# c-zhou/oatk

Measured on AMD Instinct MI355X. Metric: HiFi Gbases/s through syncasm (syncmer+syncerr) at k=1001 s=31, higher is better.
Workload: dtype u64

## Files before the change

oatk_amd/csrc/api.hip:

```cpp
#include <hip/hip_runtime.h>
#include <rocprim/device/device_radix_sort.hpp>
#include <rocprim/device/device_scan.hpp>
#include <rocprim/device/device_transform.hpp>
#include <stdio.h>
#include <stdlib.h>
#include <string.h>
#include <time.h>
#include <execinfo.h>
#include <sys/mman.h>
#include <condition_variable>
#include <mutex>
#include <string>
#include <thread>
#include <utility>
#include <vector>

#include "../../include/oatk_hip.h"
#include "common.hpp"
#include "scan_hpc.hpp"
#include "scan_syncmer.hpp"
#include "scan_syncmer_fast.hpp"
#include "kmer_hash.hpp"
#include "count.hpp"

namespace {

static int dev_alloc_log()
{
    static int on = -1;
    if (on < 0) { const char *e = getenv("OATK_DEBUG_ALLOC_LOG"); on = e && e[0] && e[0] != '0'; }
    return on;
}
static double dev_now() { struct timespec t; clock_gettime(CLOCK_MONOTONIC, &t); return (double) t.tv_sec + 1e-9 * (double) t.tv_nsec; }

constexpr size_t DM_CHUNK = 64ull << 20;
static size_t dm_min()
{
    static size_t v = 0;
    if (!v) { const char *e = getenv("OATK_DEBUG_POOL_MIN"); v = e && atoll(e) > 0? (size_t) atoll(e) : (32ull << 20); }
    return v;
}
struct ChunkPool {
    int device = -1;
    bool on = false;
    std::mutex mu;
    std::condition_variable cv;
    std::vector<hipMemGenericAllocationHandle_t> ready;
    std::vector<char> used;
    size_t created = 0, target = 0;
    bool warming = false, stop = false, failed = false;
    std::thread th;
    hipMemAllocationProp prop;
    hipMemAccessDesc acc;
    double t_wait = 0;

    bool create(hipMemGenericAllocationHandle_t *h)
    {
        const double t0 = dev_alloc_log()? dev_now() : 0;
        const hipError_t e = hipMemCreate(h, DM_CHUNK, &prop, 0);
        if (dev_alloc_log() && (e != hipSuccess || dev_now() - t0 > 0.01)) fprintf(stderr, "[oatk alloc] %.3f hipMemCreate %zu MB: %.4f s%s\n", dev_now(), DM_CHUNK >> 20, dev_now() - t0, e == hipSuccess? "" : " FAILED");
        if (e != hipSuccess) (void) hipGetLastError();
        return e == hipSuccess;
    }
    void run()
    {
        (void) hipSetDevice(device);
        for (;;) {
            {
                std::unique_lock<std::mutex> lk(mu);
                if (stop || created >= target) { warming = false; cv.notify_all(); return; }
            }
            hipMemGenericAllocationHandle_t h;
            const bool ok = create(&h);
            std::unique_lock<std::mutex> lk(mu);
            if (!ok) { failed = true, warming = false; cv.notify_all(); return; }
            ready.push_back(h), used.push_back(0), ++created;
            cv.notify_all();
        }
    }
    void warm(size_t bytes)
    {
        size_t fr = 0, tot = 0;
        if (hipMemGetInfo(&fr, &tot) == hipSuccess && bytes > fr / 10 * 7) bytes = fr / 10 * 7;
        std::unique_lock<std::mutex> lk(mu);
        const size_t want = created + bytes / DM_CHUNK;
        if (want > target) target = want;
        if (!warming && !failed && created < target) {
            if (th.joinable()) th.join();
            warming = true;
            th = std::thread([this] { run(); });
        }
    }
    bool take(hipMemGenericAllocationHandle_t *h, bool *was_used)
    {
        *was_used = false;
        {
            std::unique_lock<std::mutex> lk(mu);
            const double t0 = dev_now();
            for (;;) {
                if (!ready.empty()) { *h = ready.back(), *was_used = used.back() != 0; ready.pop_back(), used.pop_back(); t_wait += dev_now() - t0; return true; }
                if (warming && !failed && created < target) { cv.wait(lk); continue; }
                break;
            }
            t_wait += dev_now() - t0;
        }
        if (!create(h)) return false;
        std::unique_lock<std::mutex> lk(mu);
        ++created;
        return true;
    }
    void give(hipMemGenericAllocationHandle_t h)
    {
        std::unique_lock<std::mutex> lk(mu);
        ready.push_back(h), used.push_back(1);
    }
    size_t trim()
    {
        std::unique_lock<std::mutex> lk(mu);
        const size_t n = ready.size();
        for (auto h : ready) (void) hipMemRelease(h);
        ready.clear(), used.clear();
        created -= n, target = created;
        return n;
    }
    void end()
    {
        { std::unique_lock<std::mutex> lk(mu); stop = true; cv.notify_all(); }
        if (th.joinable()) th.join();
    }
};
static ChunkPool *g_pool[64];
static std::mutex g_pool_mu;
static void pools_end() { for (ChunkPool *p : g_pool) if (p) p->end(); }
static ChunkPool *pool_of_current_device()
{
    int d = -1;
    if (hipGetDevice(&d) != hipSuccess || d < 0 || d >= 64) return nullptr;
    ChunkPool *p = g_pool[d];
    return p && p->on? p : nullptr;
}
static ChunkPool *pool_for_new_buffer()
{
    ChunkPool *p = pool_of_current_device();
    if (!p) return nullptr;
    static long lo = -1, hi = -1, seq = 0;
    if (lo < 0) { const char *e = getenv("OATK_DEBUG_POOL_SEQ"); lo = 0, hi = 1L << 60; if (e) sscanf(e, "%ld:%ld", &lo, &hi); }
    const long k = seq++;
    if (dev_alloc_log()) {
        void *bt[6];
        const int nb = backtrace(bt, 6);
        char **sy = backtrace_symbols(bt, nb);
        fprintf(stderr, "[oatk alloc] decision %ld%s  <- %s <- %s <- %s\n", k, k >= lo && k < hi? "" : " (hipMalloc)", nb > 2? sy[2] : "", nb > 3? sy[3] : "", nb > 4? sy[4] : "");
        free(sy);
    }
    return k >= lo && k < hi? p : nullptr;
}

static hipError_t dev_malloc(void **p, size_t bytes)
{
    const double t0 = dev_alloc_log()? dev_now() : 0;
    hipError_t e = hipMalloc(p, bytes);
    if (e != hipSuccess) {
        ChunkPool *pl = pool_of_current_device();
        if (pl && pl->trim()) { (void) hipGetLastError(); e = hipMalloc(p, bytes); }
    }
    if (dev_alloc_log()) fprintf(stderr, "[oatk alloc] %.3f hipMalloc %10.3f MB: %.4f s%s\n", dev_now(), (double) bytes / 1e6, dev_now() - t0, e == hipSuccess? "" : " FAILED");
    {
        static int poison = -1;
        if (poison < 0) { const char *ev = getenv("OATK_DEBUG_POISON"); poison = ev && ev[0] == '1'; }
        if (poison && e == hipSuccess) { (void) hipMemset(*p, 0xA5, bytes); (void) hipDeviceSynchronize(); }
    }
    return e;
}
static void dev_free(void *p, size_t bytes)
{
    const double t0 = dev_alloc_log()? dev_now() : 0;
    (void) hipFree(p);
    if (dev_alloc_log()) fprintf(stderr, "[oatk alloc] %.3f hipFree   %10.3f MB: %.4f s\n", dev_now(), (double) bytes / 1e6, dev_now() - t0);
}

struct DevBuf {
    void *p = nullptr;
    size_t cap = 0;
    size_t va = 0;
    ChunkPool *pool = nullptr;
    bool decided = false;
    std::vector<hipMemGenericAllocationHandle_t> ch;

    static size_t up(size_t b) { return (b + DM_CHUNK - 1) / DM_CHUNK * DM_CHUNK; }
    bool vm_range(size_t bytes, hipStream_t st)
    {
        if (bytes <= va) return true;
        const size_t nva = up(bytes < (1ull << 30)? 4 * bytes + (256ull << 20) : bytes + bytes / 2 + (2ull << 30));
        void *np = nullptr;
        { const hipError_t er = hipMemAddressReserve(&np, nva, 2 << 20, nullptr, 0);
          if (er != hipSuccess) { if (dev_alloc_log()) fprintf(stderr, "[oatk alloc] hipMemAddressReserve of %.1f MB FAILED: %s\n", (double) nva / 1e6, hipGetErrorString(er)); (void) hipGetLastError(); return false; } }
        if (!ch.empty()) {
            (void) hipStreamSynchronize(st);
            (void) hipDeviceSynchronize();
            for (size_t i = 0; i < ch.size(); ++i) {
                (void) hipMemUnmap((char *) p + i * DM_CHUNK, DM_CHUNK);
                if (hipMemMap((char *) np + i * DM_CHUNK, DM_CHUNK, 0, ch[i], 0) != hipSuccess) return false;
            }
            if (hipMemSetAccess(np, ch.size() * DM_CHUNK, &pool->acc, 1) != hipSuccess) return false;
        }
        if (dev_alloc_log()) fprintf(stderr, "[oatk alloc] %.3f address range %10.3f MB (%zu pieces moved)\n", dev_now(), (double) nva / 1e6, ch.size());
        p = np, va = nva;
        return true;
    }
    bool vm_grow(size_t bytes, hipStream_t st)
    {
        const size_t want = up(bytes);
        if (!vm_range(want, st)) return false;
        const size_t have = ch.size() * DM_CHUNK;
        const double t0 = dev_alloc_log()? dev_now() : 0;
        bool any_used = false;
        while (ch.size() * DM_CHUNK < want) {
            hipMemGenericAllocationHandle_t h;
            bool was_used;
            if (!pool->take(&h, &was_used)) { if (dev_alloc_log()) fprintf(stderr, "[oatk alloc] no piece to be had\n"); break; }
            { const hipError_t er = hipMemMap((char *) p + ch.size() * DM_CHUNK, DM_CHUNK, 0, h, 0);
              if (er != hipSuccess) { if (dev_alloc_log()) fprintf(stderr, "[oatk alloc] hipMemMap FAILED: %s\n", hipGetErrorString(er)); (void) hipGetLastError(); pool->give(h); break; } }
            ch.push_back(h);
            any_used |= was_used;
        }
        const size_t now_b = ch.size() * DM_CHUNK;
        if (now_b > have) { const hipError_t er = hipMemSetAccess((char *) p + have, now_b - have, &pool->acc, 1);
                            if (er != hipSuccess) { if (dev_alloc_log()) fprintf(stderr, "[oatk alloc] hipMemSetAccess FAILED: %s\n", hipGetErrorString(er)); (void) hipGetLastError(); return false; } }
        if (any_used && now_b > have && (hipMemsetAsync((char *) p + have, 0, now_b - have, st) != hipSuccess || hipStreamSynchronize(st) != hipSuccess)) return false;
        if (dev_alloc_log()) fprintf(stderr, "[oatk alloc] %.3f pieces    %10.3f MB -> %10.3f MB: %.4f s\n", dev_now(), (double) have / 1e6, (double) now_b / 1e6, dev_now() - t0);
        cap = now_b;
        return now_b >= want;
    }
    bool ensure(size_t bytes, hipStream_t st, bool zero_new = false)
    {
        if (bytes <= cap) return true;
        if (!va && !decided) pool = bytes >= dm_min()? pool_for_new_buffer() : nullptr, decided = bytes >= dm_min();
        if (pool && p && !va) { (void) hipStreamSynchronize(st); dev_free(p, cap); p = nullptr; cap = 0; }
        if (pool) {
            if (vm_grow(bytes + bytes / 16, st)) {
                if (zero_new) (void) hipMemsetAsync(p, 0, cap, st);
                return true;
            }
            if (!ch.empty()) return false;
            pool = nullptr, p = nullptr, cap = 0, va = 0;
        }
        if (p) { (void) hipStreamSynchronize(st); dev_free(p, cap); p = nullptr; cap = 0; }
        size_t want = bytes + bytes / 8 + 256;
        if (dev_malloc(&p, want) != hipSuccess) { p = nullptr; return false; }
        cap = want;
        if (zero_new) (void) hipMemsetAsync(p, 0, want, st);
        return true;
    }
    bool grow_keep(size_t bytes, size_t used, hipStream_t st)
    {
        if (bytes <= cap) return true;
        if (!va && !decided) pool = bytes >= dm_min()? pool_for_new_buffer() : nullptr, decided = bytes >= dm_min();
        if (pool && p && !va) {
            void *old = p;
            const size_t old_cap = cap;
            p = nullptr, cap = 0;
            if (!vm_grow(bytes, st)) { release(); p = old, cap = old_cap, pool = nullptr; }
            else {
                if (used && hipMemcpyAsync(p, old, used, hipMemcpyDeviceToDevice, st) != hipSuccess) return false;
                (void) hipStreamSynchronize(st);
                dev_free(old, old_cap);
                return true;
            }
        }
        if (pool) return vm_grow(bytes, st);
        void *np = nullptr;
        size_t want = bytes + bytes / 4 + 256;
        if (dev_malloc(&np, want) != hipSuccess) return false;
        if (p && used && hipMemcpyAsync(np, p, used, hipMemcpyDeviceToDevice, st) != hipSuccess) { dev_free(np, want); return false; }
        (void) hipStreamSynchronize(st);
        if (p) dev_free(p, cap);
        p = np, cap = want;
        return true;
    }
    bool reserve(size_t bytes, size_t used, hipStream_t st)
    {
        if (bytes <= cap) return true;
        if (!va && !p && !decided) pool = bytes >= dm_min()? pool_for_new_buffer() : nullptr, decided = bytes >= dm_min();
        if (pool && (va || !p)) return vm_range(up(bytes), st);
        return grow_keep(bytes, used, st);
    }
    void release()
    {
        if (va) {
            (void) hipDeviceSynchronize();
            for (size_t i = 0; i < ch.size(); ++i) { (void) hipMemUnmap((char *) p + i * DM_CHUNK, DM_CHUNK); pool->give(ch[i]); }
            ch.clear();
            if (dev_alloc_log()) fprintf(stderr, "[oatk alloc] %.3f pieces    %10.3f MB back to the pool\n", dev_now(), (double) cap / 1e6);
            p = nullptr, cap = 0, va = 0, decided = false;
            return;
        }
        if (p) dev_free(p, cap);
        p = nullptr; cap = 0, decided = false;
    }
    template <class T> T *as() const { return (T *) p; }
};

}

struct oatk_hip_ctx {
    int device = 0;
    int n_cu = 256;
    hipStream_t stream = nullptr;
    std::string err;
    bool timing = false;
    hipEvent_t ev[OATK_T_COUNT_ + 1][2];
    bool ev_used[OATK_T_COUNT_ + 1];
    float ms[OATK_T_COUNT_];
    uint64_t hash_mask = ~0ULL;
    bool force_general = false;
    void *staging = nullptr;
    uint64_t staging_cap = 0;
    void *staging_raw = nullptr;
    uint64_t staging_raw_size = 0;
    bool ra_two_pass = false;
    int list_cap = 0;
    uint64_t import_reserve = 1u << 20;
    int ec_cap_t0 = 0, ec_cap_t1 = 0;

    const uint8_t *d_seq = nullptr;
    const uint64_t *d_off = nullptr;
    const uint32_t *d_len = nullptr;
    DevBuf in_seq, in_off, in_len;
    uint64_t n_reads = 0, seq_bytes = 0, sid0 = 0;
    int K = 0, S = 0;
    bool scanned = false, counted = false;

    DevBuf hoco_l, n_scm, n_nn, n_lrl, ho_rl, hoco_s, nbits;
    DevBuf nn_key, lrl_key, lrl_val, nn_key2, lrl_key2, lrl_val2;
    DevBuf rec_hash, rec_lo, rec_smer, rec_mpos;
    DevBuf raw_lo, raw_smer, raw_mpos, shard_cnt, shard_prefix;
    uint32_t region_cap = 0;
    DevBuf counters;
    uint32_t nn_cap = 0, lrl_cap = 0;
    uint64_t n_occ = 0, tot_nn = 0, tot_lrl = 0, n_scm_total = 0;
    uint32_t retries = 0, collisions = 0;
    bool nn_sorted_in_2 = false, lrl_sorted_in_2 = false;

    DevBuf n_scm64, scm_off, pos_hash, pos_lo, pos_smer, pos_mpos, pos_kid;
    DevBuf key_hash, key_sorted, iota, perm, head, head_idx, newclus, clus_id, bad_head, tag, tmp_perm, flags, kloc, smer_sorted, slot_rec, scm_loc;
    DevBuf scm_h, scm_s, scm_cov, scm_occ_off, scm_occ;
    DevBuf tmp;
    struct EcState *ec = nullptr;
    struct ConsState *cons = nullptr;
    struct IngState *ing = nullptr;
    struct StatState *stat = nullptr;
    struct AgState *ag = nullptr;
    struct OvlState *ovl = nullptr;
    struct RaState *ra = nullptr;
    struct RcState *rc = nullptr;
    struct MultiState *multi = nullptr;
};

#define CK(call)                                                                                   \
    do {                                                                                           \
        hipError_t e_ = (call);                                                                    \
        if (e_ != hipSuccess) {                                                                    \
            ctx->err = std::string(#call) + ": " + hipGetErrorString(e_);                          \
            return OATK_E_NODEV;                                                                   \
        }                                                                                          \
    } while (0)
#define ENSURE(buf, bytes, ...)                                                                    \
    do {                                                                                           \
        if (!ctx->buf.ensure((bytes), ctx->stream, ##__VA_ARGS__)) {                               \
            ctx->err = "hipMalloc failed for " #buf;                                               \
            return OATK_E_NOMEM;                                                                   \
        }                                                                                          \
    } while (0)

static bool debug_refuse(oatk_hip_ctx *ctx, int bit, const char *what)
{
    const char *e = getenv("OATK_DEBUG_REFUSE");
    if (!e || !(atoi(e) & bit)) return false;
    ctx->err = std::string(what) + ": refused on request (OATK_DEBUG_REFUSE)";
    return true;
}

static void t_begin(oatk_hip_ctx *ctx, int which)
{
    if (!ctx->timing) return;
    (void) hipEventRecord(ctx->ev[which][0], ctx->stream);
}
static void t_end(oatk_hip_ctx *ctx, int which)
{
    if (!ctx->timing) return;
    (void) hipEventRecord(ctx->ev[which][1], ctx->stream);
    ctx->ev_used[which] = true;
}
static void t_collect(oatk_hip_ctx *ctx, int first, int last)
{
    if (!ctx->timing) return;
    (void) hipStreamSynchronize(ctx->stream);
    for (int i = first; i <= last; ++i) {
        ctx->ms[i] = 0.f;
        if (ctx->ev_used[i]) (void) hipEventElapsedTime(&ctx->ms[i], ctx->ev[i][0], ctx->ev[i][1]);
        ctx->ev_used[i] = false;
    }
}

#include "api_ec.inc"
#include "api_graph.inc"
#include "api_cons.inc"
#include "api_ovl.inc"
#include "api_align.inc"
#include "api_racov.inc"
#include "api_ingest.inc"
#include "api_stat.inc"
#include "api_multi.inc"
#include "api_multi_tail.inc"

static void staging_free(oatk_hip_ctx *ctx)
{
    if (!ctx->staging) return;
    if (ctx->staging_raw) { (void) hipHostUnregister(ctx->staging); munmap(ctx->staging_raw, ctx->staging_raw_size); }
    else (void) hipHostFree(ctx->staging);
    ctx->staging = ctx->staging_raw = nullptr, ctx->staging_cap = ctx->staging_raw_size = 0;
}

extern "C" {

int oatk_hip_abi_version(void) { return OATK_HIP_ABI_VERSION; }

int oatk_hip_device_count(void)
{
    int n = 0;
    if (hipGetDeviceCount(&n) != hipSuccess) return 0;
    return n;
}

int oatk_hip_max_k(void) { return 8192 - 16 * oatk::SYN_NT - 16 - 64; }

oatk_hip_ctx *oatk_hip_create(int device)
{
    int n = 0;
    if (hipGetDeviceCount(&n) != hipSuccess || device < 0 || device >= n) return nullptr;
    if (hipSetDevice(device) != hipSuccess) return nullptr;
    oatk_hip_ctx *ctx = new oatk_hip_ctx();
    ctx->device = device;
    { int cu = 0; if (hipDeviceGetAttribute(&cu, hipDeviceAttributeMultiprocessorCount, device) == hipSuccess && cu > 0) ctx->n_cu = cu; }
    if (hipStreamCreateWithFlags(&ctx->stream, hipStreamNonBlocking) != hipSuccess) { delete ctx; return nullptr; }
    for (int i = 0; i <= OATK_T_COUNT_; ++i) {
        (void) hipEventCreate(&ctx->ev[i][0]);
        (void) hipEventCreate(&ctx->ev[i][1]);
        ctx->ev_used[i] = false;
    }
    memset(ctx->ms, 0, sizeof(ctx->ms));
    return ctx;
}

void oatk_hip_destroy(oatk_hip_ctx *ctx)
{
    if (!ctx) return;
    (void) hipSetDevice(ctx->device);
    (void) hipStreamSynchronize(ctx->stream);
    DevBuf *all[] = {&ctx->in_seq, &ctx->in_off, &ctx->in_len, &ctx->hoco_l, &ctx->n_scm, &ctx->n_nn, &ctx->n_lrl, &ctx->ho_rl,
                     &ctx->hoco_s, &ctx->nbits, &ctx->nn_key, &ctx->lrl_key, &ctx->lrl_val, &ctx->nn_key2, &ctx->lrl_key2,
                     &ctx->lrl_val2, &ctx->rec_hash, &ctx->rec_lo, &ctx->rec_smer, &ctx->rec_mpos, &ctx->raw_lo, &ctx->raw_smer, &ctx->raw_mpos, &ctx->shard_cnt, &ctx->shard_prefix, &ctx->counters, &ctx->n_scm64,
                     &ctx->scm_off, &ctx->pos_hash, &ctx->pos_lo, &ctx->pos_smer, &ctx->pos_mpos, &ctx->pos_kid, &ctx->key_hash,
                     &ctx->key_sorted, &ctx->iota, &ctx->perm, &ctx->head, &ctx->head_idx, &ctx->newclus, &ctx->clus_id, &ctx->kloc, &ctx->smer_sorted, &ctx->slot_rec, &ctx->scm_loc,
                     &ctx->bad_head, &ctx->tag, &ctx->tmp_perm, &ctx->flags, &ctx->scm_h, &ctx->scm_s, &ctx->scm_cov,
                     &ctx->scm_occ_off, &ctx->scm_occ, &ctx->tmp};
    for (DevBuf *b : all) b->release();
    ec_state_free(ctx);
    cons_state_free(ctx);
    ing_state_free(ctx);
    stat_state_free(ctx);
    ag_state_free(ctx);
    ovl_state_free(ctx);
    ra_state_free(ctx);
    rc_state_free(ctx);
    multi_state_free(ctx);
    for (int i = 0; i <= OATK_T_COUNT_; ++i) {
        (void) hipEventDestroy(ctx->ev[i][0]);
        (void) hipEventDestroy(ctx->ev[i][1]);
    }
    staging_free(ctx);
    (void) hipStreamDestroy(ctx->stream);
    delete ctx;
}

int oatk_hip_mem_pool(oatk_hip_ctx *ctx, uint64_t warm_bytes)
{
    if (!ctx) return OATK_E_NODEV;
    { const char *e = getenv("OATK_POOL"); if (e && e[0] == '0') return OATK_OK; }
    CK(hipSetDevice(ctx->device));
    if (ctx->device < 0 || ctx->device >= 64) return OATK_E_ARG;
    ChunkPool *pl;
    {
        std::unique_lock<std::mutex> lk(g_pool_mu);
        pl = g_pool[ctx->device];
        if (!pl) {
            int vmm = 0;
            if (hipDeviceGetAttribute(&vmm, hipDeviceAttributeVirtualMemoryManagementSupported, ctx->device) != hipSuccess || !vmm) { (void) hipGetLastError(); return OATK_OK; }
            pl = new ChunkPool();
            pl->device = ctx->device;
            memset(&pl->prop, 0, sizeof(pl->prop));
            pl->prop.type = hipMemAllocationTypePinned;
            pl->prop.location.type = hipMemLocationTypeDevice;
            pl->prop.location.id = ctx->device;
            memset(&pl->acc, 0, sizeof(pl->acc));
            pl->acc.location = pl->prop.location;
            pl->acc.flags = hipMemAccessFlagsProtReadWrite;
            static bool at_exit = false;
            if (!at_exit) { at_exit = true; atexit(pools_end); }
            pl->on = true;
            g_pool[ctx->device] = pl;
        }
    }
    if (warm_bytes) pl->warm((size_t) warm_bytes);
    return OATK_OK;
}

const char *oatk_hip_last_error(oatk_hip_ctx *ctx) { return ctx? ctx->err.c_str() : "no device context"; }
void *oatk_hip_stream(oatk_hip_ctx *ctx) { return ctx? (void *) ctx->stream : nullptr; }
int oatk_hip_sync(oatk_hip_ctx *ctx)
{
    if (!ctx) return OATK_E_NODEV;
    CK(hipStreamSynchronize(ctx->stream));
    return OATK_OK;
}
int oatk_hip_set_timing(oatk_hip_ctx *ctx, int enable)
{
    if (!ctx) return OATK_E_NODEV;
    ctx->timing = enable != 0;
    return OATK_OK;
}
int oatk_hip_get_timing(oatk_hip_ctx *ctx, float *ms, int n)
{
    if (!ctx) return OATK_E_NODEV;
    for (int i = 0; i < n && i < OATK_T_COUNT_; ++i) ms[i] = ctx->ms[i];
    return OATK_OK;
}
int oatk_hip_debug_force_general(oatk_hip_ctx *ctx, int on)
{
    if (!ctx) return OATK_E_NODEV;
    ctx->force_general = on != 0;
    return OATK_OK;
}
int oatk_hip_debug_align_two_pass(oatk_hip_ctx *ctx, int on)
{
    if (!ctx) return OATK_E_NODEV;
    ctx->ra_two_pass = on != 0;
    return OATK_OK;
}
int oatk_hip_debug_list_cap(oatk_hip_ctx *ctx, int cap)
{
    if (!ctx) return OATK_E_NODEV;
    if (cap < 0 || cap > oatk::SYF_LIST) { ctx->err = "oatk_hip_debug_list_cap: 0 <= cap <= 128"; return OATK_E_ARG; }
    ctx->list_cap = cap;
    return OATK_OK;
}
int oatk_hip_debug_hash_mask(oatk_hip_ctx *ctx, uint64_t mask)
{
    if (!ctx) return OATK_E_NODEV;
    ctx->hash_mask = mask;
    return OATK_OK;
}

__global__ void widen_kernel(const uint32_t *in, uint64_t *out, uint64_t n)
{
    uint64_t i = (uint64_t) blockIdx.x * blockDim.x + threadIdx.x;
    if (i < n) out[i] = in[i];
    if (i == n) out[i] = 0;
}

static void scan_reset_downstream(oatk_hip_ctx *ctx);

static int launch_scan_kernels(oatk_hip_ctx *ctx)
{
    using namespace oatk;
    const uint64_t n = ctx->n_reads;
    CK(hipMemsetAsync(ctx->counters.p, 0, 4 * sizeof(uint32_t), ctx->stream));
    CK(hipMemsetAsync(ctx->shard_cnt.p, 0, oatk::OATK_REC_SHARDS * sizeof(uint32_t), ctx->stream));
    HpcArgs h;
    h.seq = ctx->d_seq, h.off = ctx->d_off, h.len = ctx->d_len, h.sid0 = ctx->sid0;
    h.ho_rl = ctx->ho_rl.as<uint8_t>(), h.hoco_s = ctx->hoco_s.as<uint8_t>(), h.nbits = ctx->nbits.as<uint32_t>();
    h.hoco_l = ctx->hoco_l.as<uint32_t>(), h.n_nn = ctx->n_nn.as<uint32_t>(), h.n_lrl = ctx->n_lrl.as<uint32_t>();
    h.nn_key = ctx->nn_key.as<uint64_t>(), h.lrl_key = ctx->lrl_key.as<uint64_t>(), h.lrl_val = ctx->lrl_val.as<uint32_t>();
    h.nn_cap = ctx->nn_cap, h.lrl_cap = ctx->lrl_cap, h.counters = ctx->counters.as<uint32_t>();
    t_begin(ctx, OATK_T_HPC);
    h.n_reads = (uint32_t) n;
    constexpr int HPC_NW = 4;
    uint64_t hpc_grid = (uint64_t) ctx->n_cu * 8 * 8;
    { const char *ev = getenv("OATK_DEBUG_HPC_GRID"); if (ev && atoi(ev) > 0) hpc_grid = (uint64_t) atoi(ev); }
    if (hpc_grid * HPC_NW > n) hpc_grid = (n + HPC_NW - 1) / HPC_NW;
    unsigned hpc_dyn = 0;
    { const char *ev = getenv("OATK_DEBUG_HPC_LDS"); if (ev && atoi(ev) > 0) hpc_dyn = (unsigned) atoi(ev); }
    hipLaunchKernelGGL((hpc_pack_kernel<HPC_NW>), dim3((unsigned) (hpc_grid? hpc_grid : 1)), dim3(HPC_NW * OATK_WAVE), hpc_dyn, ctx->stream, h);
    t_end(ctx, OATK_T_HPC);

    SynArgs s;
    s.hoco_s = ctx->hoco_s.as<uint8_t>(), s.nbits = ctx->nbits.as<uint32_t>(), s.off = ctx->d_off;
    s.hoco_l = ctx->hoco_l.as<uint32_t>(), s.n_nn = ctx->n_nn.as<uint32_t>(), s.sid0 = ctx->sid0;
    s.K = ctx->K, s.S = ctx->S, s.want_n = 0, s.n_scm = ctx->n_scm.as<uint32_t>(), s.list_cap = ctx->list_cap? ctx->list_cap : SYF_LIST;
    s.rec_hash = nullptr, s.rec_lo = ctx->raw_lo.as<uint64_t>(), s.rec_smer = ctx->raw_smer.as<uint64_t>();
    s.rec_mpos = ctx->raw_mpos.as<uint32_t>(), s.region_cap = ctx->region_cap, s.shard_cnt = ctx->shard_cnt.as<uint32_t>();
    const bool small = ctx->K + 8 * SYN_NT + 8 + 64 <= 4096;
    const int fast_ring = ctx->force_general? 0 : syncmer_fast_ring(ctx->K, ctx->S);
    t_begin(ctx, OATK_T_SYNCMER);
    if (fast_ring == 4096) {
        const dim3 g((unsigned) n), b(SYN_NT);
        unsigned dyn = 0;
        { const char *ev = getenv("OATK_DEBUG_SYNCMER_LDS"); if (ev && atoi(ev) > 0) dyn = (unsigned) atoi(ev); }
#define OATK_SYF_SWITCH(S31) switch ((-(ctx->K - ctx->S)) & 7) { \
            case 0: OATK_SYF_LAUNCH(S31, 0); break; case 1: OATK_SYF_LAUNCH(S31, 1); break; case 2: OATK_SYF_LAUNCH(S31, 2); break; \
            case 3: OATK_SYF_LAUNCH(S31, 3); break; case 4: OATK_SYF_LAUNCH(S31, 4); break; case 5: OATK_SYF_LAUNCH(S31, 5); break; \
            case 6: OATK_SYF_LAUNCH(S31, 6); break; default: OATK_SYF_LAUNCH(S31, 7); break; }
        const bool two_waves = ctx->K - ctx->S < 1024 && getenv("OATK_DEBUG_SYNCMER_NT256") == nullptr;
#define OATK_SYF_LAUNCH(S31, SH) do { if (two_waves) hipLaunchKernelGGL((syncmer_fast_kernel<2048, S31, 128, SH>), g, dim3(128), dyn, ctx->stream, s); \
                                      else hipLaunchKernelGGL((syncmer_fast_kernel<4096, S31, SYN_NT, SH>), g, b, dyn, ctx->stream, s); } while (0)
        if (ctx->S == 31) OATK_SYF_SWITCH(true) else OATK_SYF_SWITCH(false)
#undef OATK_SYF_SWITCH
#undef OATK_SYF_LAUNCH
    }
    else if (small) hipLaunchKernelGGL((syncmer_kernel<8, 4096, false>), dim3((unsigned) n), dim3(SYN_NT), 0, ctx->stream, s);
    else hipLaunchKernelGGL((syncmer_kernel<16, 8192, false>), dim3((unsigned) n), dim3(SYN_NT), 0, ctx->stream, s);
    t_end(ctx, OATK_T_SYNCMER);
    uint32_t n_amb = 0;
    CK(hipMemcpyAsync(&n_amb, ctx->counters.as<uint32_t>(), 4, hipMemcpyDeviceToHost, ctx->stream));
    CK(hipStreamSynchronize(ctx->stream));
    s.want_n = 1;
    t_begin(ctx, OATK_T_SYNCMER_N);
    if (n_amb) {
        if (small) hipLaunchKernelGGL((syncmer_kernel<8, 4096, true>), dim3((unsigned) n), dim3(SYN_NT), 0, ctx->stream, s);
        else hipLaunchKernelGGL((syncmer_kernel<16, 8192, true>), dim3((unsigned) n), dim3(SYN_NT), 0, ctx->stream, s);
    }
    t_end(ctx, OATK_T_SYNCMER_N);
    CK(hipGetLastError());
    return OATK_OK;
}

int oatk_hip_scan(oatk_hip_ctx *ctx, const uint8_t *d_seq, const uint64_t *d_off, const uint32_t *d_len,
                  uint64_t n_reads, uint64_t seq_bytes, uint64_t sid0, int k, int s)
{
    if (!ctx) return OATK_E_NODEV;
    CK(hipSetDevice(ctx->device));
    if (!(s > 0 && s < 32 && k > s) || k > oatk_hip_max_k()) { ctx->err = "k/s out of range for the device scan"; return OATK_E_ARG; }
    if (seq_bytes % OATK_READ_ALIGN || n_reads >= 0xFFFFFFFFULL || sid0 + n_reads > 0xFFFFFFFFULL) { ctx->err = "bad batch geometry"; return OATK_E_ARG; }
    ctx->d_seq = d_seq, ctx->d_off = d_off, ctx->d_len = d_len;
    ctx->n_reads = n_reads, ctx->seq_bytes = seq_bytes, ctx->sid0 = sid0, ctx->K = k, ctx->S = s;
    scan_reset_downstream(ctx);
    ctx->retries = 0, ctx->collisions = 0;
    ctx->n_occ = ctx->tot_nn = ctx->tot_lrl = ctx->n_scm_total = 0;
    if (n_reads == 0) { ctx->scanned = true; return OATK_OK; }

    ENSURE(hoco_l, n_reads * 4); ENSURE(n_scm, n_reads * 4); ENSURE(n_nn, n_reads * 4); ENSURE(n_lrl, n_reads * 4);
    ENSURE(ho_rl, seq_bytes + 64);
    ENSURE(hoco_s, seq_bytes / 4 + 128 + 16 + ctx->import_reserve);
    ENSURE(nbits, seq_bytes / 8 + 128, true);
    ENSURE(counters, 64);
    if (ctx->nn_cap == 0) ctx->nn_cap = 1u << 14;
    if (ctx->lrl_cap == 0) ctx->lrl_cap = 1u << 14;
    const uint32_t NSH = oatk::OATK_REC_SHARDS;
    {
        uint64_t guess = (seq_bytes / 256 + 1024) / NSH + 256;
        if (ctx->region_cap < guess) ctx->region_cap = (uint32_t) guess;
    }
    ENSURE(shard_cnt, NSH * 4); ENSURE(shard_prefix, NSH * 8);
    uint32_t sc[oatk::OATK_REC_SHARDS];
    uint64_t spfx[oatk::OATK_REC_SHARDS];

    for (;;) {
        const size_t raw_n = (size_t) ctx->region_cap * NSH;
        ENSURE(raw_lo, raw_n * 8); ENSURE(raw_smer, raw_n * 8); ENSURE(raw_mpos, raw_n * 4);
        ENSURE(nn_key, (size_t) ctx->nn_cap * 8); ENSURE(nn_key2, (size_t) ctx->nn_cap * 8);
        ENSURE(lrl_key, (size_t) ctx->lrl_cap * 8); ENSURE(lrl_key2, (size_t) ctx->lrl_cap * 8);
        ENSURE(lrl_val, (size_t) ctx->lrl_cap * 4); ENSURE(lrl_val2, (size_t) ctx->lrl_cap * 4);
        int rc = launch_scan_kernels(ctx);
        if (rc) return rc;
        uint32_t c[4];
        CK(hipMemcpyAsync(c, ctx->counters.p, sizeof(c), hipMemcpyDeviceToHost, ctx->stream));
        CK(hipMemcpyAsync(sc, ctx->shard_cnt.p, sizeof(sc), hipMemcpyDeviceToHost, ctx->stream));
        CK(hipStreamSynchronize(ctx->stream));
        bool again = false;
        if (c[0] > ctx->nn_cap) ctx->nn_cap = c[0] + c[0] / 4, again = true;
        if (c[1] > ctx->lrl_cap) ctx->lrl_cap = c[1] + c[1] / 4, again = true;
        uint64_t tot = 0;
        uint32_t mx = 0;
        for (uint32_t i = 0; i < NSH; ++i) { spfx[i] = tot; tot += sc[i]; if (sc[i] > mx) mx = sc[i]; }
        if (mx > ctx->region_cap) ctx->region_cap = mx + mx / 4 + 16, again = true;
        if (tot > 0xFFFFFFF0ULL) { ctx->err = "more than 2^32 syncmer occurrences in one batch"; return OATK_E_ARG; }
        ctx->tot_nn = c[0], ctx->tot_lrl = c[1], ctx->n_occ = tot;
        if (!again) break;
        ++ctx->retries;
        CK(hipMemsetAsync(ctx->nbits.p, 0, ctx->nbits.cap, ctx->stream));
    }
    if (ctx->n_occ) {
        ENSURE(rec_hash, (size_t) ctx->n_occ * 8); ENSURE(rec_lo, (size_t) ctx->n_occ * 8);
        ENSURE(rec_smer, (size_t) ctx->n_occ * 8); ENSURE(rec_mpos, (size_t) ctx->n_occ * 4);
        CK(hipMemcpyAsync(ctx->shard_prefix.p, spfx, sizeof(spfx), hipMemcpyHostToDevice, ctx->stream));
        oatk::CompactArgs ca;
        ca.raw_lo = ctx->raw_lo.as<uint64_t>(), ca.raw_smer = ctx->raw_smer.as<uint64_t>(), ca.raw_mpos = ctx->raw_mpos.as<uint32_t>();
        ca.shard_cnt = ctx->shard_cnt.as<uint32_t>(), ca.shard_prefix = ctx->shard_prefix.as<uint64_t>(), ca.region_cap = ctx->region_cap;
        ca.rec_lo = ctx->rec_lo.as<uint64_t>(), ca.rec_smer = ctx->rec_smer.as<uint64_t>(), ca.rec_mpos = ctx->rec_mpos.as<uint32_t>();
        hipLaunchKernelGGL(oatk::compact_records_kernel, dim3(NSH), dim3(256), 0, ctx->stream, ca);
        CK(hipStreamSynchronize(ctx->stream));
    }
    if (ctx->timing) t_collect(ctx, OATK_T_HPC, OATK_T_SYNCMER_N);

    if (ctx->n_occ) {
        oatk::KmerHashArgs kh;
        kh.hoco_s = ctx->hoco_s.as<uint8_t>(), kh.off = ctx->d_off, kh.sid0 = ctx->sid0;
        kh.rec_lo = ctx->rec_lo.as<uint64_t>(), kh.rec_mpos = ctx->rec_mpos.as<uint32_t>(), kh.rec_hash = ctx->rec_hash.as<uint64_t>();
        kh.n_rec = (uint32_t) ctx->n_occ, kh.K = ctx->K;
        const int nw = ((ctx->K - 1) / 4 + 1 + 7) / 8;
        t_begin(ctx, OATK_T_KMER_HASH);
        hipLaunchKernelGGL(oatk::kmer_hash_kernel, dim3((unsigned) ((ctx->n_occ + KMH_REC - 1) / KMH_REC)), dim3(64), (size_t) KMH_REC * (nw + 1) * 8, ctx->stream, kh);
        t_end(ctx, OATK_T_KMER_HASH);
    }

    t_begin(ctx, OATK_T_SCAN_POST);
    ctx->nn_sorted_in_2 = ctx->lrl_sorted_in_2 = false;
    if (ctx->tot_nn > 1) {
        size_t tb = 0;
        CK(rocprim::radix_sort_keys(nullptr, tb, ctx->nn_key.as<uint64_t>(), ctx->nn_key2.as<uint64_t>(), ctx->tot_nn, 0, 64, ctx->stream));
        ENSURE(tmp, tb);
        CK(rocprim::radix_sort_keys(ctx->tmp.p, tb, ctx->nn_key.as<uint64_t>(), ctx->nn_key2.as<uint64_t>(), ctx->tot_nn, 0, 64, ctx->stream));
        ctx->nn_sorted_in_2 = true;
    }
    if (ctx->tot_lrl > 1) {
        size_t tb = 0;
        CK(rocprim::radix_sort_pairs(nullptr, tb, ctx->lrl_key.as<uint64_t>(), ctx->lrl_key2.as<uint64_t>(), ctx->lrl_val.as<uint32_t>(),
                                     ctx->lrl_val2.as<uint32_t>(), ctx->tot_lrl, 0, 64, ctx->stream));
        ENSURE(tmp, tb);
        CK(rocprim::radix_sort_pairs(ctx->tmp.p, tb, ctx->lrl_key.as<uint64_t>(), ctx->lrl_key2.as<uint64_t>(), ctx->lrl_val.as<uint32_t>(),
                                     ctx->lrl_val2.as<uint32_t>(), ctx->tot_lrl, 0, 64, ctx->stream));
        ctx->lrl_sorted_in_2 = true;
    }
    {
        ENSURE(n_scm64, (n_reads + 1) * 8); ENSURE(scm_off, (n_reads + 1) * 8);
        unsigned nb = (unsigned) ((n_reads + 1 + 255) / 256);
        hipLaunchKernelGGL(widen_kernel, dim3(nb), dim3(256), 0, ctx->stream, ctx->n_scm.as<uint32_t>(), ctx->n_scm64.as<uint64_t>(), n_reads);
        size_t tb = 0;
        CK(rocprim::exclusive_scan(nullptr, tb, ctx->n_scm64.as<uint64_t>(), ctx->scm_off.as<uint64_t>(), (uint64_t) 0, n_reads + 1,
                                   rocprim::plus<uint64_t>(), ctx->stream));
        ENSURE(tmp, tb);
        CK(rocprim::exclusive_scan(ctx->tmp.p, tb, ctx->n_scm64.as<uint64_t>(), ctx->scm_off.as<uint64_t>(), (uint64_t) 0, n_reads + 1,
                                   rocprim::plus<uint64_t>(), ctx->stream));
    }
    {
        using namespace oatk;
        size_t n = ctx->n_occ? ctx->n_occ : 1;
        ENSURE(pos_hash, n * 8); ENSURE(pos_lo, n * 8); ENSURE(pos_smer, n * 8); ENSURE(pos_mpos, n * 4);
        ENSURE(key_hash, n * 8); ENSURE(iota, n * 4);
        if (ctx->n_occ) {
            PlaceArgs p;
            p.rec_hash = ctx->rec_hash.as<uint64_t>(), p.rec_lo = ctx->rec_lo.as<uint64_t>(), p.rec_smer = ctx->rec_smer.as<uint64_t>();
            p.rec_mpos = ctx->rec_mpos.as<uint32_t>(), p.n_rec = (uint32_t) ctx->n_occ, p.sid0 = ctx->sid0;
            p.scm_off = ctx->scm_off.as<uint64_t>(), p.hash_mask = ctx->hash_mask;
            p.pos_hash = ctx->pos_hash.as<uint64_t>(), p.pos_lo = ctx->pos_lo.as<uint64_t>(), p.pos_smer = ctx->pos_smer.as<uint64_t>();
            p.pos_mpos = ctx->pos_mpos.as<uint32_t>(), p.key_hash = ctx->key_hash.as<uint64_t>(), p.iota = ctx->iota.as<uint32_t>();
            t_begin(ctx, OATK_T_COUNT_PLACE);
            hipLaunchKernelGGL(place_records_kernel, dim3((unsigned) ((ctx->n_occ + 255) / 256)), dim3(256), 0, ctx->stream, p);
            t_end(ctx, OATK_T_COUNT_PLACE);
        }
    }
    t_end(ctx, OATK_T_SCAN_POST);
    CK(hipGetLastError());
    CK(hipStreamSynchronize(ctx->stream));
    if (ctx->timing) { t_collect(ctx, OATK_T_SCAN_POST, OATK_T_COUNT_PLACE); t_collect(ctx, OATK_T_KMER_HASH, OATK_T_KMER_HASH); }
    ctx->scanned = true;
    return OATK_OK;
}

__global__ void append_rebase_kernel(const uint64_t *src, uint64_t *dst, uint64_t n, uint64_t add)
{
    uint64_t i = (uint64_t) blockIdx.x * blockDim.x + threadIdx.x;
    if (i < n) dst[i] = src[i] + add;
}
__global__ void append_iota_kernel(uint32_t *iota, uint64_t first, uint64_t n)
{
    uint64_t i = (uint64_t) blockIdx.x * blockDim.x + threadIdx.x;
    if (i < n) iota[first + i] = (uint32_t) (first + i);
}

static void scan_reset_downstream(oatk_hip_ctx *ctx)
{
    ctx->scanned = ctx->counted = false;
    if (ctx->ec) ctx->ec->done = ctx->ec->marked = ctx->ec->graph_resident = ctx->ec->global = false;
    if (ctx->cons) ctx->cons->done = false;
    if (ctx->ag) ctx->ag->done = false;
    if (ctx->ovl) ctx->ovl->done = false;
    if (ctx->ra) ctx->ra->done = false;
    if (ctx->multi) ctx->multi->merged = ctx->multi->ec_done = false;
}

int oatk_hip_device(oatk_hip_ctx *ctx) { return ctx? ctx->device : -1; }

int oatk_hip_d2d(oatk_hip_ctx *ctx, void *d_dst, const void *d_src, uint64_t bytes)
{
    if (!ctx) return OATK_E_NODEV;
    if (bytes == 0) return OATK_OK;
    CK(hipSetDevice(ctx->device));
    CK(hipMemcpyAsync(d_dst, d_src, bytes, hipMemcpyDeviceToDevice, ctx->stream));
    CK(hipStreamSynchronize(ctx->stream));
    return OATK_OK;
}

int oatk_hip_scan_begin(oatk_hip_ctx *ctx, uint64_t sid0, int k, int s)
{
    if (!ctx) return OATK_E_NODEV;
    CK(hipSetDevice(ctx->device));
    if (!(s > 0 && s < 32 && k > s) || k > oatk_hip_max_k()) { ctx->err = "k/s out of range for the device scan"; return OATK_E_ARG; }
    scan_reset_downstream(ctx);
    ctx->d_seq = nullptr, ctx->d_off = nullptr, ctx->d_len = nullptr;
    ctx->n_reads = 0, ctx->seq_bytes = 0, ctx->sid0 = sid0, ctx->K = k, ctx->S = s;
    ctx->retries = 0, ctx->collisions = 0;
    ctx->n_occ = ctx->tot_nn = ctx->tot_lrl = ctx->n_scm_total = 0;
    ctx->nn_sorted_in_2 = ctx->lrl_sorted_in_2 = false;
    ctx->scanned = true;
    return OATK_OK;
}

#define KEEP(buf, bytes, used)                                                                     \
    do {                                                                                           \
        if (!ctx->buf.grow_keep((bytes), (used), ctx->stream)) {                                   \
            ctx->err = "hipMalloc failed for " #buf " (append)";                                   \
            return OATK_E_NOMEM;                                                                   \
        }                                                                                          \
    } while (0)

static int append_ensure(oatk_hip_ctx *ctx, uint64_t nr, uint64_t sb, uint64_t occ, uint64_t nn, uint64_t lrl)
{
    const uint64_t n0 = ctx->n_reads, b0 = ctx->seq_bytes, o0 = ctx->n_occ;
    KEEP(in_off, (nr + 1) * 8, n0 * 8);
    KEEP(hoco_l, nr * 4 + 4, n0 * 4); KEEP(n_scm, nr * 4 + 4, n0 * 4); KEEP(n_nn, nr * 4 + 4, n0 * 4); KEEP(n_lrl, nr * 4 + 4, n0 * 4);
    KEEP(ho_rl, sb + 64, b0);
    KEEP(hoco_s, sb / 4 + 128 + 16 + ctx->import_reserve, b0 / 4 + 64);
    KEEP(scm_off, (nr + 1) * 8, (n0 + 1) * 8);
    KEEP(pos_hash, occ * 8 + 8, o0 * 8); KEEP(pos_lo, occ * 8 + 8, o0 * 8); KEEP(pos_smer, occ * 8 + 8, o0 * 8); KEEP(pos_mpos, occ * 4 + 4, o0 * 4);
    KEEP(key_hash, occ * 8 + 8, o0 * 8); KEEP(iota, occ * 4 + 4, o0 * 4);
    KEEP(nn_key, nn * 8 + 8, ctx->tot_nn * 8); KEEP(lrl_key, lrl * 8 + 8, ctx->tot_lrl * 8); KEEP(lrl_val, lrl * 4 + 4, ctx->tot_lrl * 4);
    return OATK_OK;
}

int oatk_hip_scan_reserve(oatk_hip_ctx *ctx, uint64_t seq_bytes, uint64_t n_reads, uint64_t n_occ)
{
    if (!ctx) return OATK_E_NODEV;
    CK(hipSetDevice(ctx->device));
    if (!ctx->scanned || ctx->d_seq) { ctx->err = "oatk_hip_scan_reserve: call oatk_hip_scan_begin first"; return OATK_E_STATE; }
    seq_bytes = (seq_bytes + 63) & ~63ULL;
    if (pool_of_current_device()) {
        const uint64_t sb = ctx->seq_bytes + seq_bytes;
        if (!ctx->ho_rl.reserve(sb + 64, ctx->seq_bytes, ctx->stream) || !ctx->hoco_s.reserve(sb / 4 + 128 + 16 + ctx->import_reserve, ctx->seq_bytes / 4 + 64, ctx->stream)) {
            ctx->err = "oatk_hip_scan_reserve: no address range for the batch";
            return OATK_E_NOMEM;
        }
        return OATK_OK;
    }
    return append_ensure(ctx, ctx->n_reads + n_reads, ctx->seq_bytes + seq_bytes, ctx->n_occ + n_occ, ctx->tot_nn, ctx->tot_lrl);
}

int oatk_hip_scan_append(oatk_hip_ctx *ctx, oatk_hip_ctx *src)
{
    if (!ctx || !src) return OATK_E_NODEV;
    CK(hipSetDevice(ctx->device));
    if (ctx == src || ctx->device != src->device) { ctx->err = "oatk_hip_scan_append: the piece must be another handle on the same device"; return OATK_E_ARG; }
    if (!ctx->scanned || ctx->d_seq) { ctx->err = "oatk_hip_scan_append: call oatk_hip_scan_begin first"; return OATK_E_STATE; }
    if (!src->scanned) { ctx->err = "oatk_hip_scan_append: the piece holds no scan"; return OATK_E_STATE; }
    const uint64_t n0 = ctx->n_reads, n1 = src->n_reads, b0 = ctx->seq_bytes, b1 = src->seq_bytes, o0 = ctx->n_occ, o1 = src->n_occ;
    if (n1 == 0) return OATK_OK;
    if (src->K != ctx->K || src->S != ctx->S) { ctx->err = "oatk_hip_scan_append: the piece was scanned with another k / s"; return OATK_E_ARG; }
    if (src->sid0 != ctx->sid0 + n0) { ctx->err = "oatk_hip_scan_append: the piece's first read id must continue the batch"; return OATK_E_ARG; }
    if (n0 + n1 >= 0xFFFFFFFFULL || o0 + o1 > 0xFFFFFFF0ULL) { ctx->err = "oatk_hip_scan_append: batch too large"; return OATK_E_ARG; }
    scan_reset_downstream(ctx);
    ctx->scanned = true;
    { int rc = append_ensure(ctx, n0 + n1, b0 + b1, o0 + o1, ctx->tot_nn + src->tot_nn, ctx->tot_lrl + src->tot_lrl); if (rc) return rc; }
    if (hipStreamSynchronize(src->stream) != hipSuccess) { ctx->err = "oatk_hip_scan_append: the piece's stream failed"; return OATK_E_NODEV; }
    hipStream_t st = ctx->stream;
    auto blocks = [](uint64_t n) { return dim3((unsigned) ((n + 255) / 256 > 0? (n + 255) / 256 : 1)); };
    auto d2d = [&](void *dst, const void *from, size_t bytes) { return bytes? hipMemcpyAsync(dst, from, bytes, hipMemcpyDeviceToDevice, st) : hipSuccess; };
    CK(d2d(ctx->ho_rl.as<uint8_t>() + b0, src->ho_rl.p, b1));
    CK(d2d(ctx->hoco_s.as<uint8_t>() + b0 / 4, src->hoco_s.p, b1 / 4 + 64));
    CK(d2d(ctx->hoco_l.as<uint32_t>() + n0, src->hoco_l.p, n1 * 4)); CK(d2d(ctx->n_scm.as<uint32_t>() + n0, src->n_scm.p, n1 * 4));
    CK(d2d(ctx->n_nn.as<uint32_t>() + n0, src->n_nn.p, n1 * 4)); CK(d2d(ctx->n_lrl.as<uint32_t>() + n0, src->n_lrl.p, n1 * 4));
    hipLaunchKernelGGL(append_rebase_kernel, blocks(n1), dim3(256), 0, st, src->d_off, ctx->in_off.as<uint64_t>() + n0, n1, b0);
    hipLaunchKernelGGL(append_rebase_kernel, blocks(n1 + 1), dim3(256), 0, st, src->scm_off.as<uint64_t>(), ctx->scm_off.as<uint64_t>() + n0, n1 + 1, o0);
    if (o1) {
        CK(d2d(ctx->pos_hash.as<uint64_t>() + o0, src->pos_hash.p, o1 * 8)); CK(d2d(ctx->pos_lo.as<uint64_t>() + o0, src->pos_lo.p, o1 * 8));
        CK(d2d(ctx->pos_smer.as<uint64_t>() + o0, src->pos_smer.p, o1 * 8)); CK(d2d(ctx->pos_mpos.as<uint32_t>() + o0, src->pos_mpos.p, o1 * 4));
        CK(d2d(ctx->key_hash.as<uint64_t>() + o0, src->key_hash.p, o1 * 8));
        hipLaunchKernelGGL(append_iota_kernel, blocks(o1), dim3(256), 0, st, ctx->iota.as<uint32_t>(), o0, o1);
    }
    CK(d2d(ctx->nn_key.as<uint64_t>() + ctx->tot_nn, src->nn_sorted_in_2? src->nn_key2.p : src->nn_key.p, src->tot_nn * 8));
    CK(d2d(ctx->lrl_key.as<uint64_t>() + ctx->tot_lrl, src->lrl_sorted_in_2? src->lrl_key2.p : src->lrl_key.p, src->tot_lrl * 8));
    CK(d2d(ctx->lrl_val.as<uint32_t>() + ctx->tot_lrl, src->lrl_sorted_in_2? src->lrl_val2.p : src->lrl_val.p, src->tot_lrl * 4));
    CK(hipGetLastError());
    CK(hipStreamSynchronize(st));
    ctx->d_off = ctx->in_off.as<uint64_t>();
    ctx->n_reads = n0 + n1, ctx->seq_bytes = b0 + b1, ctx->n_occ = o0 + o1;
    ctx->tot_nn += src->tot_nn, ctx->tot_lrl += src->tot_lrl;
    ctx->retries += src->retries;
    return OATK_OK;
}

int oatk_hip_scan_host(oatk_hip_ctx *ctx, const uint8_t *h_seq, const uint64_t *h_off, const uint32_t *h_len,
                       uint64_t n_reads, uint64_t seq_bytes, uint64_t sid0, int k, int s)
{
    if (!ctx) return OATK_E_NODEV;
    CK(hipSetDevice(ctx->device));
    ENSURE(in_seq, seq_bytes + 64); ENSURE(in_off, (n_reads + 1) * 8); ENSURE(in_len, (n_reads + 1) * 4);
    if (seq_bytes) CK(hipMemcpyAsync(ctx->in_seq.p, h_seq, seq_bytes, hipMemcpyHostToDevice, ctx->stream));
    if (n_reads) {
        CK(hipMemcpyAsync(ctx->in_off.p, h_off, n_reads * 8, hipMemcpyHostToDevice, ctx->stream));
        CK(hipMemcpyAsync(ctx->in_len.p, h_len, n_reads * 4, hipMemcpyHostToDevice, ctx->stream));
    }
    return oatk_hip_scan(ctx, ctx->in_seq.as<uint8_t>(), ctx->in_off.as<uint64_t>(), ctx->in_len.as<uint32_t>(), n_reads, seq_bytes, sid0, k, s);
}

int oatk_hip_count(oatk_hip_ctx *ctx)
{
    using namespace oatk;
    if (!ctx) return OATK_E_NODEV;
    if (!ctx->scanned) { ctx->err = "count before scan"; return OATK_E_STATE; }
    CK(hipSetDevice(ctx->device));
    ctx->counted = false;
    ctx->n_scm_total = 0;
    if (ctx->multi) ctx->multi->merged = ctx->multi->ec_done = false;
    const uint64_t n = ctx->n_occ;
    if (n == 0) { ctx->counted = true; return OATK_OK; }
    const unsigned nb = (unsigned) ((n + 255) / 256);

    ENSURE(key_sorted, n * 8); ENSURE(perm, n * 4); ENSURE(head, n * 4); ENSURE(head_idx, n * 4); ENSURE(newclus, n * 4); ENSURE(kloc, n * 8);
    if (ctx->seq_bytes >> 4 >= 0xFFFFFFFFULL) { ctx->err = "batch too large for 32-bit hoco word indices (64 GB of bases)"; return OATK_E_ARG; }
    ENSURE(clus_id, n * 4); ENSURE(bad_head, n * 4); ENSURE(tag, n * 4); ENSURE(tmp_perm, n * 4); ENSURE(flags, 64);
    ENSURE(pos_kid, n * 8); ENSURE(scm_occ, n * 8);
    CK(hipMemsetAsync(ctx->flags.p, 0, 64, ctx->stream));

    bool full_sort = getenv("OATK_DEBUG_FULL_SORT") != nullptr || n < (1ull << 22);
sort_again:
    t_begin(ctx, OATK_T_COUNT_SORT);
    {
        const unsigned lo_bit = full_sort? 0u : (unsigned) OATK_SORT_LOW_BITS;
        size_t tb = 0;
        CK(rocprim::radix_sort_pairs(nullptr, tb, ctx->key_hash.as<uint64_t>(), ctx->key_sorted.as<uint64_t>(), ctx->iota.as<uint32_t>(),
                                     ctx->perm.as<uint32_t>(), n, lo_bit, 64, ctx->stream));
        ENSURE(tmp, tb);
        CK(rocprim::radix_sort_pairs(ctx->tmp.p, tb, ctx->key_hash.as<uint64_t>(), ctx->key_sorted.as<uint64_t>(), ctx->iota.as<uint32_t>(),
                                     ctx->perm.as<uint32_t>(), n, lo_bit, 64, ctx->stream));
        if (!full_sort) {
            uint32_t *owner = ctx->head.as<uint32_t>();
            CK(hipMemsetAsync(owner, 0xFF, n * 4, ctx->stream));
            hipLaunchKernelGGL(sort_repair_find_kernel, dim3(nb), dim3(256), 0, ctx->stream, ctx->key_sorted.as<uint64_t>(), (uint32_t) n, owner, ctx->flags.as<uint32_t>());
            hipLaunchKernelGGL(sort_repair_kernel, dim3(nb), dim3(256), 0, ctx->stream, ctx->key_sorted.as<uint64_t>(), ctx->perm.as<uint32_t>(), (uint32_t) n, owner,
                               ctx->flags.as<uint32_t>());
        }
    }
    t_end(ctx, OATK_T_COUNT_SORT);

    t_begin(ctx, OATK_T_COUNT_GROUP);
    GroupArgs g;
    g.sorted_key = ctx->key_sorted.as<uint64_t>(), g.perm = ctx->perm.as<uint32_t>(), g.n_rec = (uint32_t) n;
    g.pos_lo = ctx->pos_lo.as<uint64_t>(), g.pos_mpos = ctx->pos_mpos.as<uint32_t>(), g.hoco_s = ctx->hoco_s.as<uint8_t>();
    g.off = ctx->d_off, g.sid0 = ctx->sid0, g.K = ctx->K;
    g.head = ctx->head.as<uint32_t>(), g.head_idx = ctx->head_idx.as<uint32_t>(), g.newclus = ctx->newclus.as<uint32_t>();
    g.loc = ctx->kloc.as<uint64_t>();
    ENSURE(smer_sorted, n * 8);
    g.pos_smer = ctx->pos_smer.as<uint64_t>(), g.occ_sorted = ctx->scm_occ.as<uint64_t>(), g.smer_sorted = ctx->smer_sorted.as<uint64_t>();
    g.flags = ctx->flags.as<uint32_t>();
    ENSURE(slot_rec, n * 32);
    g.slot_rec = ctx->slot_rec.as<uint4>();
    hipLaunchKernelGGL(pack_slots_kernel, dim3(nb), dim3(256), 0, ctx->stream, g);
    hipLaunchKernelGGL(pair_sum_kernel, dim3(2048), dim3(256), 0, ctx->stream, ctx->key_hash.as<uint64_t>(), (const uint32_t *) nullptr, (uint32_t) n, ctx->flags.as<uint32_t>(), 8);
    hipLaunchKernelGGL(pair_sum_kernel, dim3(2048), dim3(256), 0, ctx->stream, ctx->key_sorted.as<uint64_t>(), ctx->perm.as<uint32_t>(), (uint32_t) n, ctx->flags.as<uint32_t>(), 12);
    hipLaunchKernelGGL(heads_only_kernel, dim3(nb), dim3(256), 0, ctx->stream, g);
    {
        size_t tb = 0;
        CK(rocprim::inclusive_scan(nullptr, tb, ctx->head_idx.as<uint32_t>(), ctx->head_idx.as<uint32_t>(), n, rocprim::maximum<uint32_t>(), ctx->stream));
        ENSURE(tmp, tb);
        CK(rocprim::inclusive_scan(ctx->tmp.p, tb, ctx->head_idx.as<uint32_t>(), ctx->head_idx.as<uint32_t>(), n, rocprim::maximum<uint32_t>(), ctx->stream));
    }
    uint32_t n_scm = 0;
    FinishArgs f;
    auto ids = [&]() -> int {
        size_t tb = 0;
        CK(rocprim::inclusive_scan(nullptr, tb, ctx->newclus.as<uint32_t>(), ctx->clus_id.as<uint32_t>(), n, rocprim::plus<uint32_t>(), ctx->stream));
        ENSURE(tmp, tb);
        CK(rocprim::inclusive_scan(ctx->tmp.p, tb, ctx->newclus.as<uint32_t>(), ctx->clus_id.as<uint32_t>(), n, rocprim::plus<uint32_t>(), ctx->stream));
        uint32_t last_id = 0;
        CK(hipMemcpyAsync(&last_id, ctx->clus_id.as<uint32_t>() + (n - 1), 4, hipMemcpyDeviceToHost, ctx->stream));
        CK(hipStreamSynchronize(ctx->stream));
        n_scm = last_id;
        ENSURE(scm_h, (size_t) n_scm * 8); ENSURE(scm_s, (size_t) n_scm * 8); ENSURE(scm_cov, (size_t) n_scm * 4); ENSURE(scm_loc, (size_t) n_scm * 8);
        ENSURE(scm_occ_off, ((size_t) n_scm + 1) * 8);
        f.perm = ctx->perm.as<uint32_t>(), f.newclus = ctx->newclus.as<uint32_t>(), f.clus_id = ctx->clus_id.as<uint32_t>(), f.n_rec = (uint32_t) n;
        f.sorted_key = ctx->key_sorted.as<uint64_t>(), f.smer_sorted = ctx->smer_sorted.as<uint64_t>();
        f.loc = ctx->kloc.as<uint64_t>(), f.scm_loc = ctx->scm_loc.as<uint64_t>();
        f.scm_h = ctx->scm_h.as<uint64_t>(), f.scm_s = ctx->scm_s.as<uint64_t>(), f.scm_occ_off = ctx->scm_occ_off.as<uint64_t>();
        f.scm_occ = ctx->scm_occ.as<uint64_t>(), f.pos_kid = ctx->pos_kid.as<uint64_t>(), f.flags = ctx->flags.as<uint32_t>();
        return OATK_OK;
    };
    { int rc = ids(); if (rc) return rc; }
    hipLaunchKernelGGL(gather_finish_kernel, dim3(nb), dim3(256), 0, ctx->stream, g, f, ctx->clus_id.as<uint32_t>(), n_scm);
    CK(hipMemsetAsync(ctx->bad_head.p, 0, n * 4, ctx->stream));
    hipLaunchKernelGGL(verify_group_kernel, dim3((unsigned) ((n + 8 * OATK_VG_STRIP - 1) / (8 * OATK_VG_STRIP))), dim3(256), 0, ctx->stream, g, ctx->bad_head.as<uint32_t>());
    CK(rocprim::transform(ctx->clus_id.as<uint32_t>(), ctx->clus_id.as<uint32_t>(), n, [] __device__(uint32_t v) { return v - 1u; }, ctx->stream));
    uint32_t fl[16];
    CK(hipMemcpyAsync(fl, ctx->flags.p, sizeof(fl), hipMemcpyDeviceToHost, ctx->stream));
    CK(hipStreamSynchronize(ctx->stream));
    const bool sort_bad = fl[4] != 0 || memcmp(fl + 8, fl + 12, 16) != 0 || (!full_sort && getenv("OATK_DEBUG_SORT_DISTRUST") != nullptr);
    if (sort_bad && full_sort) {
        t_end(ctx, OATK_T_COUNT_GROUP);
        ctx->err = "the device sort returned something that is not its input in order (rocPRIM radix_sort_pairs): refusing to build the syncmer table from it";
        return OATK_E_NODEV;
    }
    if ((fl[3] || sort_bad) && !full_sort) {
        t_end(ctx, OATK_T_COUNT_GROUP);
        CK(hipMemsetAsync(ctx->flags.p, 0, 64, ctx->stream));
        full_sort = true;
        goto sort_again;
    }
    if (fl[0]) {
        ctx->collisions = 1;
        hipLaunchKernelGGL(split_collisions_kernel, dim3(nb), dim3(256), 0, ctx->stream, g, ctx->bad_head.as<uint32_t>(), ctx->perm.as<uint32_t>(),
                           ctx->tag.as<uint32_t>(), ctx->tmp_perm.as<uint32_t>());
        hipLaunchKernelGGL(regather_kernel, dim3(nb), dim3(256), 0, ctx->stream, g);
        { int rc = ids(); if (rc) return rc; }
        CK(rocprim::transform(ctx->clus_id.as<uint32_t>(), ctx->clus_id.as<uint32_t>(), n, [] __device__(uint32_t v) { return v - 1u; }, ctx->stream));
        hipLaunchKernelGGL(finish_heads_kernel, dim3(nb), dim3(256), 0, ctx->stream, f, n_scm);
    }
    hipLaunchKernelGGL(check_smer_kernel, dim3(nb), dim3(256), 0, ctx->stream, f);
    hipLaunchKernelGGL(cov_kernel, dim3((n_scm + 255) / 256), dim3(256), 0, ctx->stream, ctx->scm_occ_off.as<uint64_t>(), ctx->scm_cov.as<uint32_t>(), n_scm);
    t_end(ctx, OATK_T_COUNT_GROUP);
    CK(hipGetLastError());
    CK(hipMemcpyAsync(fl, ctx->flags.p, sizeof(fl), hipMemcpyDeviceToHost, ctx->stream));
    CK(hipStreamSynchronize(ctx->stream));
    if (ctx->timing) t_collect(ctx, OATK_T_COUNT_SORT, OATK_T_COUNT_GROUP);
    if (fl[2]) { ctx->err = "hash group with too many distinct k-mers"; return OATK_E_SPLIT; }
    if (debug_refuse(ctx, 4, "oatk_hip_count")) return OATK_E_SPLIT;
    if (fl[1]) { ctx->err = "identical kmers have different smers"; return OATK_E_SMER; }
    ctx->n_scm_total = n_scm;
    ctx->counted = true;
    return OATK_OK;
}

int oatk_hip_info(oatk_hip_ctx *ctx, oatk_hip_info_t *out)
{
    if (!ctx) return OATK_E_NODEV;
    out->n_reads = ctx->n_reads, out->seq_bytes = ctx->seq_bytes, out->sid0 = ctx->sid0;
    out->k = ctx->K, out->s = ctx->S;
    out->n_occ = ctx->n_occ, out->n_nn = ctx->tot_nn, out->n_lrl = ctx->tot_lrl;
    out->n_scm = ctx->n_scm_total;
    out->scan_retries = ctx->retries, out->collisions = ctx->collisions;
    return OATK_OK;
}

int oatk_hip_buffer(oatk_hip_ctx *ctx, int which, const void **d_ptr, uint64_t *bytes)
{
    if (!ctx) return OATK_E_NODEV;
    if (which >= OATK_BUF_INGEST_SEQ && which <= OATK_BUF_INGEST_HDR) return ing_buffer(ctx, which, d_ptr, bytes);
    if (which >= OATK_BUF_MG_H && which <= OATK_BUF_MG_LCOV) return multi_buffer(ctx, which, d_ptr, bytes);
    if (which >= OATK_BUF_MG_G_H && which <= OATK_BUF_MG_POS_GKID) return multi_tail_buffer(ctx, which, d_ptr, bytes);
    if (!ctx->scanned) { ctx->err = "no resident scan"; return OATK_E_STATE; }
    const uint64_t n = ctx->n_reads, occ = ctx->n_occ, ns = ctx->n_scm_total;
    const void *p = nullptr;
    uint64_t b = 0;
    switch (which) {
        case OATK_BUF_HOCO_L: p = ctx->hoco_l.p, b = n * 4; break;
        case OATK_BUF_N_SCM: p = ctx->n_scm.p, b = n * 4; break;
        case OATK_BUF_N_NN: p = ctx->n_nn.p, b = n * 4; break;
        case OATK_BUF_N_LRL: p = ctx->n_lrl.p, b = n * 4; break;
        case OATK_BUF_HO_RL: p = ctx->ho_rl.p, b = ctx->seq_bytes; break;
        case OATK_BUF_HOCO_S: p = ctx->hoco_s.p, b = ctx->seq_bytes / 4 + 64; break;
        case OATK_BUF_NN_KEY: p = ctx->nn_sorted_in_2? ctx->nn_key2.p : ctx->nn_key.p, b = ctx->tot_nn * 8; break;
        case OATK_BUF_LRL_KEY: p = ctx->lrl_sorted_in_2? ctx->lrl_key2.p : ctx->lrl_key.p, b = ctx->tot_lrl * 8; break;
        case OATK_BUF_LRL_VAL: p = ctx->lrl_sorted_in_2? ctx->lrl_val2.p : ctx->lrl_val.p, b = ctx->tot_lrl * 4; break;
        case OATK_BUF_SCM_OFF: p = ctx->scm_off.p, b = (n + 1) * 8; break;
        case OATK_BUF_POS_MPOS: p = ctx->pos_mpos.p, b = occ * 4; break;
        case OATK_BUF_POS_SMER: p = ctx->pos_smer.p, b = occ * 8; break;
        case OATK_BUF_POS_HASH: p = ctx->pos_hash.p, b = occ * 8; break;
        default:
            if (!ctx->counted) { ctx->err = "count results requested before oatk_hip_count"; return OATK_E_STATE; }
            switch (which) {
                case OATK_BUF_POS_KID: p = ctx->pos_kid.p, b = occ * 8; break;
                case OATK_BUF_SCM_H: p = ctx->scm_h.p, b = ns * 8; break;
                case OATK_BUF_SCM_S: p = ctx->scm_s.p, b = ns * 8; break;
                case OATK_BUF_SCM_COV: p = ctx->scm_cov.p, b = ns * 4; break;
                case OATK_BUF_SCM_OCC_OFF: p = ctx->scm_occ_off.p, b = (ns + 1) * 8; break;
                case OATK_BUF_SCM_OCC: p = ctx->scm_occ.p, b = occ * 8; break;
                default:
                    if (which >= OATK_BUF_CONS_SEL && which <= OATK_BUF_CONS_TOT) return cons_buffer(ctx, which, d_ptr, bytes);
                    if (which >= OATK_BUF_AG_SCM_DEL && which <= OATK_BUF_AG_ARC_LINK) return ag_buffer(ctx, which, d_ptr, bytes);
                    if (which >= OATK_BUF_OVL_KEY && which <= OATK_BUF_OVL_TAIL) return ovl_buffer(ctx, which, d_ptr, bytes);
                    if (which >= OATK_BUF_RA_ALN_SID && which <= OATK_BUF_RA_SKIPPED) return ra_buffer(ctx, which, d_ptr, bytes);
                    if (which >= OATK_BUF_INGEST_SEQ && which <= OATK_BUF_INGEST_HDR) return ing_buffer(ctx, which, d_ptr, bytes);
                    return ec_buffer(ctx, which, d_ptr, bytes);
            }
    }
    *d_ptr = p, *bytes = b;
    return OATK_OK;
}

void *oatk_hip_staging(oatk_hip_ctx *ctx, uint64_t bytes)
{
    if (!ctx || hipSetDevice(ctx->device) != hipSuccess) return nullptr;
    if (bytes <= ctx->staging_cap) return ctx->staging;
    staging_free(ctx);
    const uint64_t HP = 2ull << 20, want = (bytes + HP - 1) & ~(HP - 1);
    void *raw = mmap(nullptr, want + HP, PROT_READ | PROT_WRITE, MAP_PRIVATE | MAP_ANONYMOUS, -1, 0);
    if (raw != MAP_FAILED) {
        uint8_t *base = (uint8_t *) (((uintptr_t) raw + HP - 1) & ~(uintptr_t) (HP - 1));
        (void) madvise(base, want, MADV_HUGEPAGE);
        const int nt = want >= (256ull << 20)? 8 : 1;
        std::vector<std::thread> th;
        for (int t = 1; t < nt; ++t) th.emplace_back([=] { for (uint64_t o = want / nt * t; o < (t + 1 == nt? want : want / nt * (t + 1)); o += 4096) *(volatile uint8_t *) (base + o) = 0; });
        for (uint64_t o = 0; o < want / nt; o += 4096) *(volatile uint8_t *) (base + o) = 0;
        for (auto &x : th) x.join();
        if (hipHostRegister(base, want, hipHostRegisterDefault) == hipSuccess) {
            ctx->staging = base, ctx->staging_cap = want, ctx->staging_raw = raw, ctx->staging_raw_size = want + HP;
            return ctx->staging;
        }
        (void) hipGetLastError();
        munmap(raw, want + HP);
    }
    if (hipHostMalloc(&ctx->staging, bytes, hipHostMallocDefault) != hipSuccess) { ctx->staging = nullptr; ctx->err = "hipHostMalloc failed (staging)"; return nullptr; }
    ctx->staging_cap = bytes;
    return ctx->staging;
}

int oatk_hip_host_register(oatk_hip_ctx *ctx, void *p, uint64_t bytes)
{
    if (!ctx) return OATK_E_NODEV;
    if (!p || bytes == 0) return OATK_E_ARG;
    CK(hipSetDevice(ctx->device));
    CK(hipHostRegister(p, bytes, hipHostRegisterDefault));
    return OATK_OK;
}

int oatk_hip_host_unregister(oatk_hip_ctx *ctx, void *p)
{
    if (!ctx) return OATK_E_NODEV;
    CK(hipSetDevice(ctx->device));
    CK(hipHostUnregister(p));
    return OATK_OK;
}

int oatk_hip_d2h(oatk_hip_ctx *ctx, void *h_dst, const void *d_src, uint64_t bytes)
{
    if (!ctx) return OATK_E_NODEV;
    if (bytes == 0) return OATK_OK;
    CK(hipSetDevice(ctx->device));
    CK(hipMemcpyAsync(h_dst, d_src, bytes, hipMemcpyDeviceToHost, ctx->stream));
    CK(hipStreamSynchronize(ctx->stream));
    return OATK_OK;
}

int oatk_hip_d2h_async(oatk_hip_ctx *ctx, void *h_dst, const void *d_src, uint64_t bytes)
{
    if (!ctx) return OATK_E_NODEV;
    if (bytes == 0) return OATK_OK;
    CK(hipSetDevice(ctx->device));
    CK(hipMemcpyAsync(h_dst, d_src, bytes, hipMemcpyDeviceToHost, ctx->stream));
    return OATK_OK;
}

int oatk_hip_h2d_async(oatk_hip_ctx *ctx, void *d_dst, const void *h_src, uint64_t bytes)
{
    if (!ctx) return OATK_E_NODEV;
    if (bytes == 0) return OATK_OK;
    CK(hipSetDevice(ctx->device));
    CK(hipMemcpyAsync(d_dst, h_src, bytes, hipMemcpyHostToDevice, ctx->stream));
    return OATK_OK;
}

}
```

oatk_amd/csrc/common.hpp:

```cpp
#pragma once
#include <hip/hip_runtime.h>
#include <stdint.h>

#define OATK_WAVE 64

namespace oatk {

__device__ __forceinline__ uint32_t nt4_code(uint32_t ch)
{
    uint32_t up = ch & 0xDFu;
    uint32_t t = up - 0x41u;
    bool letter = t < 32u && ((0x00180045u >> t) & 1u);
    uint32_t code = (up >> 1) & 3u;
    code ^= code >> 1;
    return ch < 4u ? ch : (letter ? code : 4u);
}

__device__ __forceinline__ uint64_t hash64(uint64_t x, uint64_t mask)
{
    x = (~x + (x << 21)) & mask;
    x ^= x >> 24;
    x = (x + (x << 3) + (x << 8)) & mask;
    x ^= x >> 14;
    x = (x + (x << 2) + (x << 4)) & mask;
    x ^= x >> 28;
    x = (x + (x << 31)) & mask;
    return x;
}

__device__ __forceinline__ uint64_t hash64_s31(uint64_t x)
{
    uint32_t lo = (uint32_t) x, hi = (uint32_t) (x >> 32);
    uint64_t p;
    p = (uint64_t) lo * 0x1FFFFFu + 0xFFFFFFFFFFFFFFFFull;
    hi = (uint32_t) (p >> 32) + (hi << 21) - hi, lo = (uint32_t) p;
    { const uint32_t t = __builtin_amdgcn_alignbit(hi, lo, 24), u = __builtin_amdgcn_ubfe(hi, 24, 6); lo ^= t, hi ^= u; }
    p = (uint64_t) lo * 265u;
    hi = hi * 265u + (uint32_t) (p >> 32), lo = (uint32_t) p;
    { const uint32_t t = __builtin_amdgcn_alignbit(hi, lo, 14), u = __builtin_amdgcn_ubfe(hi, 14, 16); lo ^= t, hi ^= u; }
    p = (uint64_t) hi << 32 | lo;
    {
        uint64_t p5;
        asm("v_lshl_add_u64 %0, %1, 2, %1" : "=v"(p5) : "v"(p));
        asm("v_lshl_add_u64 %0, %1, 4, %2" : "=v"(p) : "v"(p), "v"(p5));
    }
    hi = (uint32_t) (p >> 32), lo = (uint32_t) p;
    { const uint32_t t = __builtin_amdgcn_alignbit(hi, lo, 28), u = __builtin_amdgcn_ubfe(hi, 28, 2); lo ^= t, hi ^= u; }
    p = (uint64_t) lo * 0x80000001u;
    hi = (hi + (uint32_t) (p >> 32)) & 0x3FFFFFFFu, lo = (uint32_t) p;
    return (uint64_t) hi << 32 | lo;
}

__device__ __forceinline__ uint64_t hash64_s31_left(uint64_t x4)
{
    uint32_t lo = (uint32_t) x4 & ~3u, hi = (uint32_t) (x4 >> 32);
    uint64_t p;
    p = (uint64_t) lo * 0x1FFFFFu + 0xFFFFFFFFFFFFFFFCull;
    hi = (uint32_t) (p >> 32) + (hi << 21) - hi, lo = (uint32_t) p;
    { const uint32_t t = __builtin_amdgcn_alignbit(hi, lo, 24) & ~3u, u = hi >> 24; lo ^= t, hi ^= u; }
    p = (uint64_t) lo * 265u;
    hi = hi * 265u + (uint32_t) (p >> 32), lo = (uint32_t) p;
    { const uint32_t t = __builtin_amdgcn_alignbit(hi, lo, 14) & ~3u, u = hi >> 14; lo ^= t, hi ^= u; }
    p = (uint64_t) hi << 32 | lo;
    {
        uint64_t p5;
        asm("v_lshl_add_u64 %0, %1, 2, %1" : "=v"(p5) : "v"(p));
        asm("v_lshl_add_u64 %0, %1, 4, %2" : "=v"(p) : "v"(p), "v"(p5));
    }
    hi = (uint32_t) (p >> 32), lo = (uint32_t) p;
    { const uint32_t t = __builtin_amdgcn_alignbit(hi, lo, 28) & ~3u, u = hi >> 28; lo ^= t, hi ^= u; }
    hi += __builtin_amdgcn_alignbit(hi, lo, 1);
    return (uint64_t) hi << 32 | lo;
}

__device__ __forceinline__ uint64_t revcomp32(uint64_t x)
{
    uint32_t lo = (uint32_t) x, hi = (uint32_t) (x >> 32);
    uint32_t rlo = __builtin_bitreverse32(hi), rhi = __builtin_bitreverse32(lo);
    uint64_t r = (uint64_t) rhi << 32 | rlo;
    r = ((r >> 1) & 0x5555555555555555ULL) | ((r & 0x5555555555555555ULL) << 1);
    return ~r;
}

__device__ __forceinline__ uint64_t bswap64(uint64_t x) { return __builtin_bswap64(x); }

#define OATK_MURMUR_M 0xc6a4a7935bd1e995ULL
#define OATK_MURMUR_SEED 1234ULL

__device__ __forceinline__ uint64_t murmur_mix_word(uint64_t w)
{
    w *= OATK_MURMUR_M;
    w ^= w >> 47;
    w *= OATK_MURMUR_M;
    return w;
}

__device__ __forceinline__ uint32_t wave_incl_sum(uint32_t v, int lane)
{
#pragma unroll
    for (int d = 1; d < OATK_WAVE; d <<= 1) {
        uint32_t o = __shfl_up(v, d);
        if (lane >= d) v += o;
    }
    return v;
}

__device__ __forceinline__ int32_t wave_incl_max(int32_t v, int lane)
{
#pragma unroll
    for (int d = 1; d < OATK_WAVE; d <<= 1) {
        int32_t o = __shfl_up(v, d);
        if (lane >= d) v = v > o? v : o;
    }
    return v;
}

}
```

oatk_amd/csrc/count.hpp:

```cpp
#pragma once
#include "common.hpp"

namespace oatk {

struct CompactArgs {
    const uint64_t *raw_lo, *raw_smer;
    const uint32_t *raw_mpos;
    const uint32_t *shard_cnt;
    const uint64_t *shard_prefix;
    uint32_t region_cap;
    uint64_t *rec_lo, *rec_smer;
    uint32_t *rec_mpos;
};

__global__ __launch_bounds__(256) void compact_records_kernel(CompactArgs a)
{
    const uint32_t sh = blockIdx.x, n = a.shard_cnt[sh];
    const size_t src = (size_t) sh * a.region_cap;
    const uint64_t dst = a.shard_prefix[sh];
    for (uint32_t i = threadIdx.x; i < n; i += blockDim.x) {
        a.rec_lo[dst + i] = a.raw_lo[src + i];
        a.rec_smer[dst + i] = a.raw_smer[src + i];
        a.rec_mpos[dst + i] = a.raw_mpos[src + i];
    }
}

struct PlaceArgs {
    const uint64_t *rec_hash, *rec_lo, *rec_smer;
    const uint32_t *rec_mpos;
    uint32_t n_rec;
    uint64_t sid0;
    const uint64_t *scm_off;
    uint64_t hash_mask;
    uint64_t *pos_hash, *pos_lo, *pos_smer;
    uint32_t *pos_mpos;
    uint64_t *key_hash;
    uint32_t *iota;
};

__global__ void place_records_kernel(PlaceArgs a)
{
    uint32_t i = blockIdx.x * blockDim.x + threadIdx.x;
    if (i >= a.n_rec) return;
    uint64_t lo = a.rec_lo[i];
    uint64_t rd = (lo >> 32) - a.sid0;
    uint64_t p = a.scm_off[rd] + ((uint32_t) lo >> 1);
    a.pos_hash[p] = a.rec_hash[i];
    a.key_hash[p] = a.rec_hash[i] & a.hash_mask;
    a.pos_lo[p] = lo;
    a.pos_smer[p] = a.rec_smer[i];
    a.pos_mpos[p] = a.rec_mpos[i];
    a.iota[p] = (uint32_t) p;
}

__device__ __forceinline__ uint64_t kmer_word_global(const uint32_t *hs32, uint32_t pos, uint32_t rev, int K, int wd)
{
    int32_t t = rev? (int32_t) pos + K - 32 - 32 * wd : (int32_t) pos + 32 * wd;
    int nb = K - 32 * wd;
    nb = nb > 32? 32 : nb;
    int32_t wi = t >> 4;
    uint32_t sh = ((uint32_t) t & 15u) * 2u;
    uint32_t w0, w1, w2;
    if (wi >= 0) {
        struct __attribute__((packed, aligned(4))) W3 { uint32_t a, b, c; };
        const W3 v = *(const W3 *) (hs32 + wi);
        w0 = __builtin_bswap32(v.a), w1 = __builtin_bswap32(v.b), w2 = __builtin_bswap32(v.c);
    } else {
        w0 = 0u;
        w1 = wi + 1 >= 0? __builtin_bswap32(hs32[wi + 1]) : 0u;
        w2 = wi + 2 >= 0? __builtin_bswap32(hs32[wi + 2]) : 0u;
    }
    uint64_t hi = (uint64_t) w0 << 32 | w1;
    uint64_t V = sh? (hi << sh) | ((uint64_t) w2 >> (32u - sh)) : hi;
    if (rev) V = revcomp32(V);
    if (nb < 32) V &= ~0ULL << (64 - 2 * nb);
    return V;
}

struct GroupArgs {
    const uint64_t *sorted_key;
    const uint32_t *perm;
    uint32_t n_rec;
    const uint64_t *pos_lo;
    const uint32_t *pos_mpos;
    const uint8_t *hoco_s;
    const uint64_t *off;
    uint64_t sid0;
    int K;
    uint32_t *head;
    uint32_t *head_idx;
    uint32_t *newclus;
    uint32_t *flags;
    uint64_t *loc;
    const uint64_t *pos_smer;
    uint64_t *occ_sorted, *smer_sorted;
    uint4 *slot_rec;
};

__global__ void pack_slots_kernel(GroupArgs a)
{
    uint32_t p = blockIdx.x * blockDim.x + threadIdx.x;
    if (p >= a.n_rec) return;
    const uint64_t lo = a.pos_lo[p], sm = a.pos_smer[p];
    const uint64_t loc = ((a.off[(lo >> 32) - a.sid0] >> 4) << 32) | a.pos_mpos[p];
    a.slot_rec[2 * (size_t) p] = make_uint4((uint32_t) lo, (uint32_t) (lo >> 32), (uint32_t) sm, (uint32_t) (sm >> 32));
    a.slot_rec[2 * (size_t) p + 1] = make_uint4((uint32_t) loc, (uint32_t) (loc >> 32), 0u, 0u);
}

#define OATK_SORT_LOW_BITS 24
#define OATK_SORT_REPAIR_MAX 4096u
__device__ __forceinline__ bool sort_repair_boundary(const uint64_t *key, uint32_t n, uint32_t i, uint32_t &start, uint32_t *flags)
{
    if (i == 0 || i >= n) return false;
    const uint64_t k = key[i], kp = key[i - 1];
    if ((k >> OATK_SORT_LOW_BITS) != (kp >> OATK_SORT_LOW_BITS) || k == kp) return false;
    uint32_t s = i - 1;
    while (s > 0 && (key[s - 1] >> OATK_SORT_LOW_BITS) == (k >> OATK_SORT_LOW_BITS)) {
        --s;
        if (i - s > OATK_SORT_REPAIR_MAX) { flags[3] = 1u; return false; }
    }
    start = s;
    return true;
}
__global__ void sort_repair_find_kernel(const uint64_t *key, uint32_t n, uint32_t *owner, uint32_t *flags)
{
    const uint32_t i = blockIdx.x * blockDim.x + threadIdx.x;
    uint32_t s;
    if (sort_repair_boundary(key, n, i, s, flags)) atomicMin(&owner[s], i);
    if (i > 0 && i < n && (key[i] >> OATK_SORT_LOW_BITS) < (key[i - 1] >> OATK_SORT_LOW_BITS)) flags[3] = 1u;
}
__global__ void sort_repair_kernel(uint64_t *key, uint32_t *perm, uint32_t n, uint32_t *owner, uint32_t *flags)
{
    const uint32_t i = blockIdx.x * blockDim.x + threadIdx.x;
    uint32_t s;
    if (!sort_repair_boundary(key, n, i, s, flags) || owner[s] != i) return;
    const uint64_t top = key[i] >> OATK_SORT_LOW_BITS;
    uint32_t e = i + 1;
    while (e < n && (key[e] >> OATK_SORT_LOW_BITS) == top) {
        ++e;
        if (e - s > OATK_SORT_REPAIR_MAX) { flags[3] = 1u; return; }
    }
    for (uint32_t a = i; a < e; ++a) {
        const uint64_t kk = key[a];
        const uint32_t pp = perm[a];
        uint32_t b = a;
        while (b > s && key[b - 1] > kk) { key[b] = key[b - 1], perm[b] = perm[b - 1]; --b; }
        key[b] = kk, perm[b] = pp;
    }
}

__device__ __forceinline__ void pair_sums(uint64_t key, uint32_t slot, uint64_t &s0, uint64_t &s1)
{
    uint64_t x = key ^ ((uint64_t) slot * 0x9E3779B97F4A7C15ULL);
    x ^= x >> 32; x *= 0xD6E8FEB86659FD93ULL; x ^= x >> 32;
    s0 = x;
    x *= 0xD6E8FEB86659FD93ULL; x ^= x >> 29; x += key;
    s1 = x;
}
__global__ __launch_bounds__(256) void pair_sum_kernel(const uint64_t *key, const uint32_t *perm, uint32_t n, uint32_t *flags, int at)
{
    __shared__ uint64_t part[2][4];
    uint64_t s0 = 0, s1 = 0;
    bool inv = false;
    const uint64_t stride = (uint64_t) gridDim.x * blockDim.x;
    for (uint64_t i0 = (uint64_t) blockIdx.x * blockDim.x + threadIdx.x; i0 < n; i0 += 4 * stride) {
        uint64_t k[4], kp[4];
        uint32_t v[4];
#pragma unroll
        for (int u = 0; u < 4; ++u) {
            const uint64_t i = i0 + u * stride;
            const bool in = i < n;
            k[u] = in? key[i] : 0, v[u] = in? (perm? perm[i] : (uint32_t) i) : 0, kp[u] = in && perm && i? key[i - 1] : 0;
        }
#pragma unroll
        for (int u = 0; u < 4; ++u) {
            if (i0 + u * stride >= n) continue;
            uint64_t a, b;
            pair_sums(k[u], v[u], a, b);
            s0 += a, s1 += b;
            if (k[u] < kp[u]) inv = true;
        }
    }
    #pragma unroll
    for (int d = 32; d > 0; d >>= 1) s0 += __shfl_xor(s0, d), s1 += __shfl_xor(s1, d);
    if ((threadIdx.x & 63u) == 0) part[0][threadIdx.x >> 6] = s0, part[1][threadIdx.x >> 6] = s1;
    if (inv) flags[4] = 1u;
    __syncthreads();
    if (threadIdx.x == 0) {
        atomicAdd((unsigned long long *) (flags + at), (unsigned long long) (part[0][0] + part[0][1] + part[0][2] + part[0][3]));
        atomicAdd((unsigned long long *) (flags + at + 2), (unsigned long long) (part[1][0] + part[1][1] + part[1][2] + part[1][3]));
    }
}

__global__ void heads_only_kernel(GroupArgs a)
{
    uint32_t i = blockIdx.x * blockDim.x + threadIdx.x;
    if (i >= a.n_rec) return;
    const uint32_t h = i == 0 || a.sorted_key[i] != a.sorted_key[i - 1];
    a.head[i] = h;
    a.newclus[i] = h;
    a.head_idx[i] = h? i : 0u;
}

__global__ void mark_heads_kernel(GroupArgs a)
{
    uint32_t i = blockIdx.x * blockDim.x + threadIdx.x;
    if (i >= a.n_rec) return;
    uint32_t h = i == 0 || a.sorted_key[i] != a.sorted_key[i - 1];
    a.head[i] = h;
    a.newclus[i] = h;
    a.head_idx[i] = h? i : 0u;
    const uint32_t p = a.perm[i];
    const uint4 r0 = a.slot_rec[2 * (size_t) p], r1 = a.slot_rec[2 * (size_t) p + 1];
    a.loc[i] = (uint64_t) r1.y << 32 | r1.x;
    a.occ_sorted[i] = (uint64_t) r0.y << 32 | r0.x, a.smer_sorted[i] = (uint64_t) r0.w << 32 | r0.z;
}
__global__ void regather_kernel(GroupArgs a)
{
    uint32_t i = blockIdx.x * blockDim.x + threadIdx.x;
    if (i >= a.n_rec) return;
    const uint32_t p = a.perm[i];
    const uint4 r0 = a.slot_rec[2 * (size_t) p], r1 = a.slot_rec[2 * (size_t) p + 1];
    a.loc[i] = (uint64_t) r1.y << 32 | r1.x;
    a.occ_sorted[i] = (uint64_t) r0.y << 32 | r0.x, a.smer_sorted[i] = (uint64_t) r0.w << 32 | r0.z;
}

#ifndef OATK_VG_STRIP
#define OATK_VG_STRIP 8
#endif
#ifndef OATK_VFY_WAVES
#define OATK_VFY_WAVES 1
#endif
__global__ __launch_bounds__(256, OATK_VFY_WAVES) void verify_group_kernel(GroupArgs a, uint32_t *bad_head)
{
    const uint32_t hl = threadIdx.x & 31, half0 = threadIdx.x & 32;
    const uint32_t i0 = (uint32_t) OATK_VG_STRIP * (blockIdx.x * (blockDim.x >> 5) + (threadIdx.x >> 5));
    uint32_t my_h = 0;
    uint64_t my_lp = 0, my_lq = 0;
    bool my_live = false;
    if (hl < OATK_VG_STRIP) {
        const uint32_t i = i0 + hl;
        my_live = i < a.n_rec && !a.head[i];
        if (my_live) {
            my_h = a.head_idx[i];
            my_lp = a.loc[i];
            my_lq = a.loc[my_h];
        }
    }
    const uint64_t live_mask = (__ballot(my_live) >> half0) & ((1ULL << OATK_VG_STRIP) - 1ULL);
    if (live_mask == 0) return;
    const uint32_t *hs32 = (const uint32_t *) a.hoco_s;
    const int nw = (a.K + 31) / 32;
    uint32_t diff = 0;
    const uint32_t first_live = (uint32_t) __builtin_ctzll(live_mask);
    const uint64_t lq0 = (uint64_t) __shfl((long long) my_lq, (int) (half0 + first_live));
    const bool one_head = __ballot(my_live && my_lq != lq0) == 0;
    for (int w0 = 0; w0 < nw; w0 += 32) {
        const int wd = w0 + (int) hl;
        const bool in = wd < nw;
        uint64_t p[OATK_VG_STRIP], q[OATK_VG_STRIP];
        if (one_head) {
            const uint64_t q0 = in? kmer_word_global(hs32 + (lq0 >> 32), (uint32_t) lq0 >> 1, (uint32_t) lq0 & 1u, a.K, wd) : 0;
#pragma unroll
            for (int r = 0; r < OATK_VG_STRIP; ++r) {
                const uint64_t lp = (uint64_t) __shfl((long long) my_lp, (int) (half0 + r));
                const bool live = in && ((live_mask >> r) & 1u);
                p[r] = live? kmer_word_global(hs32 + (lp >> 32), (uint32_t) lp >> 1, (uint32_t) lp & 1u, a.K, wd) : q0;
            }
#pragma unroll
            for (int r = 0; r < OATK_VG_STRIP; ++r) diff |= (uint32_t) (p[r] != q0) << r;
        } else {
#pragma unroll
            for (int r = 0; r < OATK_VG_STRIP; ++r) {
                const uint64_t lp = (uint64_t) __shfl((long long) my_lp, (int) (half0 + r)), lq = (uint64_t) __shfl((long long) my_lq, (int) (half0 + r));
                const bool live = in && ((live_mask >> r) & 1u);
                p[r] = live? kmer_word_global(hs32 + (lp >> 32), (uint32_t) lp >> 1, (uint32_t) lp & 1u, a.K, wd) : 0;
                q[r] = live? kmer_word_global(hs32 + (lq >> 32), (uint32_t) lq >> 1, (uint32_t) lq & 1u, a.K, wd) : 0;
            }
#pragma unroll
            for (int r = 0; r < OATK_VG_STRIP; ++r) diff |= (uint32_t) (p[r] != q[r]) << r;
        }
    }
#pragma unroll
    for (int r = 0; r < OATK_VG_STRIP; ++r) {
        const uint64_t bad = (__ballot((diff >> r) & 1u) >> half0) & 0xFFFFFFFFULL;
        if (bad && hl == (uint32_t) r) a.flags[0] = 1u, bad_head[my_h] = 1u;
    }
}

#define OATK_MAX_SPLIT 16
__global__ void split_collisions_kernel(GroupArgs a, const uint32_t *bad_head, uint32_t *perm_rw, uint32_t *tag, uint32_t *tmp_perm)
{
    uint32_t i = blockIdx.x * blockDim.x + threadIdx.x;
    if (i >= a.n_rec || !a.head[i] || !bad_head[i]) return;
    uint32_t e = i + 1;
    while (e < a.n_rec && !a.head[e]) ++e;
    const int nw = (a.K + 31) / 32;
    uint32_t rep[OATK_MAX_SPLIT], nclus = 0;
    for (uint32_t t = i; t < e; ++t) {
        uint32_t p = perm_rw[t];
        uint64_t lo_p = a.pos_lo[p];
        const uint32_t *hs_p = (const uint32_t *) (a.hoco_s + (a.off[(lo_p >> 32) - a.sid0] >> 2));
        uint32_t mp = a.pos_mpos[p], c;
        for (c = 0; c < nclus; ++c) {
            uint32_t q = perm_rw[rep[c]];
            uint64_t lo_q = a.pos_lo[q];
            const uint32_t *hs_q = (const uint32_t *) (a.hoco_s + (a.off[(lo_q >> 32) - a.sid0] >> 2));
            uint32_t mq = a.pos_mpos[q];
            bool same = true;
            for (int wd = 0; wd < nw && same; ++wd)
                same = kmer_word_global(hs_p, mp >> 1, mp & 1u, a.K, wd) == kmer_word_global(hs_q, mq >> 1, mq & 1u, a.K, wd);
            if (same) break;
        }
        if (c == nclus) {
            if (nclus == OATK_MAX_SPLIT) { a.flags[2] = 1u; return; }
            rep[nclus++] = t;
        }
        tag[t] = c;
    }
    uint32_t w = i;
    for (uint32_t c = 0; c < nclus; ++c) {
        bool first = true;
        for (uint32_t t = i; t < e; ++t)
            if (tag[t] == c) {
                tmp_perm[w] = perm_rw[t];
                a.newclus[w] = first? 1u : 0u;
                first = false;
                ++w;
            }
    }
    for (uint32_t t = i; t < e; ++t) perm_rw[t] = tmp_perm[t];
}

struct FinishArgs {
    const uint32_t *perm;
    const uint32_t *newclus;
    const uint32_t *clus_id;
    uint32_t n_rec;
    const uint64_t *sorted_key, *smer_sorted;
    uint64_t *scm_h, *scm_s;
    uint64_t *scm_occ_off;
    uint64_t *scm_occ;
    const uint64_t *loc;
    uint64_t *scm_loc;
    uint64_t *pos_kid;
    uint32_t *flags;
};

__global__ void finish_heads_kernel(FinishArgs a, uint32_t n_scm)
{
    uint32_t i = blockIdx.x * blockDim.x + threadIdx.x;
    if (i >= a.n_rec) return;
    uint32_t p = a.perm[i], id = a.clus_id[i];
    a.pos_kid[p] = (uint64_t) id << 1;
    if (a.newclus[i]) {
        a.scm_h[id] = a.sorted_key[i];
        a.scm_s[id] = a.smer_sorted[i];
        a.scm_occ_off[id] = i;
        a.scm_loc[id] = a.loc[i];
    }
    if (i == a.n_rec - 1) a.scm_occ_off[n_scm] = a.n_rec;
}

__global__ void gather_finish_kernel(GroupArgs g, FinishArgs a, const uint32_t *clus_id1, uint32_t n_scm)
{
    uint32_t i = blockIdx.x * blockDim.x + threadIdx.x;
    if (i >= a.n_rec) return;
    const uint32_t p = g.perm[i], id = clus_id1[i] - 1u;
    const uint4 r0 = g.slot_rec[2 * (size_t) p], r1 = g.slot_rec[2 * (size_t) p + 1];
    const uint64_t loc = (uint64_t) r1.y << 32 | r1.x, smer = (uint64_t) r0.w << 32 | r0.z;
    g.loc[i] = loc;
    g.occ_sorted[i] = (uint64_t) r0.y << 32 | r0.x, g.smer_sorted[i] = smer;
    a.pos_kid[p] = (uint64_t) id << 1;
    if (g.newclus[i]) {
        a.scm_h[id] = a.sorted_key[i];
        a.scm_s[id] = smer;
        a.scm_occ_off[id] = i;
        a.scm_loc[id] = loc;
    }
    if (i == a.n_rec - 1) a.scm_occ_off[n_scm] = a.n_rec;
}

__global__ void check_smer_kernel(FinishArgs a)
{
    uint32_t i = blockIdx.x * blockDim.x + threadIdx.x;
    if (i >= a.n_rec) return;
    uint32_t id = a.clus_id[i];
    if (a.smer_sorted[i] != a.scm_s[id]) a.flags[1] = 1u;
}

__global__ void cov_kernel(const uint64_t *occ_off, uint32_t *cov, uint32_t n_scm)
{
    uint32_t i = blockIdx.x * blockDim.x + threadIdx.x;
    if (i < n_scm) cov[i] = (uint32_t) (occ_off[i + 1] - occ_off[i]);
}

}
```

oatk_amd/csrc/ec.hpp:

```cpp
#pragma once
#include "common.hpp"

namespace oatk {

#define EC_FAILURE 0
#define EC_SUCCESS 1
#define EC_AMBISNQ 2
#define EC_AMBISEQ 3
#define EC_MAX_DFS_PATH 10000
#define EC_MIN_ERR_SEQ_LEN 10
#define EC_MIN_ERR_BASE 6
#define EC_NONE 0xFFFFFFFFFFFFFFFFULL

struct EcGraph {
    uint64_t n_vtx, n_arc;
    const uint64_t *idx_p;
    const uint32_t *idx_n;
    const uint64_t *arc_v, *arc_w;
    const uint32_t *arc_ls, *arc_cov;
    uint8_t *arc_del;
    uint8_t *scm_del;
    const uint32_t *scm_cov;
    const uint64_t *scm_s;
    const uint64_t *vtx_hs_off;
    const uint32_t *vtx_mpos;
    const uint8_t *other;
};

struct EcReads {
    uint64_t n_reads, sid0;
    int K;
    const uint8_t *hoco_s;
    const uint64_t *off;
    const uint32_t *hoco_l;
    const uint64_t *scm_off;
    const uint64_t *k_mer;
    const uint32_t *m_pos;
};

__global__ void ec_mark_kernel(EcGraph g, uint32_t err_mer_c, uint32_t max_err_c, uint32_t err_arc_c, double max_arc_f)
{
    uint64_t i = (uint64_t) blockIdx.x * blockDim.x + threadIdx.x;
    if (i >= g.n_vtx) return;
    if (g.scm_del[i] || g.scm_cov[i] >= max_err_c) return;
    if (g.scm_cov[i] < err_mer_c) { g.scm_del[i] = 1; return; }
    const uint32_t nv = g.scm_cov[i];
    int b[2] = {-1, -1};
    for (int k = 0; k < 2; ++k) {
        const uint64_t v = i << 1 | (uint64_t) k, p = g.idx_p[v];
        const uint32_t na = g.idx_n[v];
        uint32_t live = 0;
        for (uint32_t j = 0; j < na; ++j) live += !g.arc_del[p + j];
        if (!live && !(g.other && g.other[v])) continue;
        b[k] = 0;
        for (uint32_t j = 0; j < na; ++j) {
            if (g.arc_del[p + j]) continue;
            const uint32_t nw = g.scm_cov[g.arc_w[p + j] >> 1], mn = nv < nw? nv : nw, ac = g.arc_cov[p + j];
            if (ac >= err_arc_c && (double) ac >= (double) mn * max_arc_f) { b[k] = 1; break; }
        }
    }
    if (!b[0] || !b[1]) g.scm_del[i] = 1;
}

__global__ void ec_arc_del_kernel(EcGraph g)
{
    uint64_t a = (uint64_t) blockIdx.x * blockDim.x + threadIdx.x;
    if (a >= g.n_arc) return;
    if (g.scm_del[g.arc_v[a] >> 1] || g.scm_del[g.arc_w[a] >> 1]) g.arc_del[a] = 1;
}

#define EC_NO_SRC 0xFFFFFFFFFFFFFFFFULL
__global__ void ec_vtx_src_kernel(uint64_t n_local, const uint64_t *scm_loc, const uint32_t *l2g, uint64_t *vtx_hs_off, uint32_t *vtx_mpos)
{
    uint64_t i = (uint64_t) blockIdx.x * blockDim.x + threadIdx.x;
    if (i >= n_local) return;
    const uint64_t loc = scm_loc[i], v = l2g? l2g[i] : i;
    vtx_hs_off[v] = (loc >> 32) << 2;
    vtx_mpos[v] = (uint32_t) loc;
}
__global__ void ec_remap_kernel(uint64_t n, const uint64_t *k_mer, const uint32_t *l2g, uint64_t *out)
{
    uint64_t i = (uint64_t) blockIdx.x * blockDim.x + threadIdx.x;
    if (i < n) out[i] = (uint64_t) l2g[k_mer[i] >> 1] << 1 | (k_mer[i] & 1ULL);
}

__device__ __forceinline__ uint32_t hoco_base(const uint8_t *hs, uint32_t p)
{
    return (hs[p >> 2] >> (((p & 3u) ^ 3u) << 1)) & 3u;
}

struct EcBlock {
    uint64_t beg_utg, end_utg;
    uint32_t beg_pos;
    int32_t l;
    int32_t beg, end;
    int32_t r;
};

template <class FB, class FC>
__device__ int ec_blocks(const uint8_t *scm_del, const uint64_t *km, const uint32_t *mp, int32_t n, uint32_t hoco_l, int K, FB on_block, FC on_copy)
{
    int32_t beg = -1, end, nb = 0;
    bool updated = true;
    for (;;) {
        uint32_t beg_pos = beg < 1? 0u : (mp[beg - 1] >> 1) + (uint32_t) K;
        beg_pos += EC_MIN_ERR_SEQ_LEN;
        for (end = beg + 1; end < n; ++end)
            if (!scm_del[km[end] >> 1] && !(km[end] & 1ULL) && (mp[end] >> 1) >= beg_pos) break;
        if (beg >= 0 || end < n) {
            EcBlock b;
            if (beg < 0) {
                beg = end;
                b.beg_utg = (km[beg] & ~1ULL) | (uint64_t) !(mp[beg] & 1u);
                b.beg_pos = 0, b.end_utg = EC_NONE, b.l = (int32_t) (mp[beg] >> 1), b.r = 1;
            } else {
                --beg;
                b.beg_utg = (km[beg] & ~1ULL) | (mp[beg] & 1u);
                b.beg_pos = (mp[beg] >> 1) + (uint32_t) K;
                if (end >= n) b.end_utg = EC_NONE, b.l = (int32_t) hoco_l - (int32_t) b.beg_pos;
                else b.end_utg = (km[end] & ~1ULL) | (mp[end] & 1u), b.l = (int32_t) (mp[end] >> 1) - (int32_t) b.beg_pos;
                b.r = 0;
            }
            b.beg = beg, b.end = end;
            on_block(nb, b);
            ++nb;
        } else {
            updated = false;
        }
        for (beg = end + 1; beg < n; ++beg)
            if (scm_del[km[beg] >> 1] || (km[end] & 1ULL)) break;
        if (beg > n) break;
        on_copy(end, beg);
    }
    return updated? nb : -1;
}

struct EcBlockOut {
    uint32_t status;
    uint32_t np;
    uint64_t path_off;
    uint32_t flags;
    uint32_t short_block;
    uint32_t tried, n_path;
    uint32_t wf_steps, wf_diag;
    uint32_t ticks, tier;
};

struct __attribute__((aligned(32))) EcLiveArc {
    uint32_t w, ls;
    uint32_t hs16, mpos;
    uint32_t lp, ln;
    uint32_t pad[2];
};
struct EcLive {
    const uint32_t *idx_p, *idx_n;
    const EcLiveArc *arc;
};

struct __attribute__((aligned(16))) EcWork {
    uint64_t beg_utg, end_utg;
    uint32_t read, beg_pos;
    int32_t l, r;
    uint32_t hs16;
    uint32_t lp, ln;
    uint32_t pad;
};

__global__ void ec_live_flag_kernel(uint64_t n_arc, const uint8_t *arc_del, uint32_t *live)
{
    uint64_t a = (uint64_t) blockIdx.x * blockDim.x + threadIdx.x;
    if (a < n_arc) live[a] = !arc_del[a];
}
__global__ void ec_live_idx_kernel(uint64_t n_ovtx, const uint64_t *idx_p, const uint32_t *idx_n, const uint64_t *live_off, uint32_t *lidx_p, uint32_t *lidx_n, uint32_t *branches)
{
    uint64_t v = (uint64_t) blockIdx.x * blockDim.x + threadIdx.x;
    if (v >= n_ovtx) return;
    const uint32_t n = idx_n[v];
    const uint64_t p = n? live_off[idx_p[v]] : 0;
    const uint32_t ln = n? (uint32_t) (live_off[idx_p[v] + n] - p) : 0u;
    lidx_p[v] = (uint32_t) p, lidx_n[v] = ln;
    if (ln > 1u && *(volatile uint32_t *) branches == 0u) atomicOr(branches, 1u);
}
__global__ void ec_live_arc_kernel(uint64_t n_arc, const uint8_t *arc_del, const uint64_t *live_off, const uint64_t *arc_w, const uint32_t *arc_ls,
                                   const uint64_t *vtx_hs_off, const uint32_t *vtx_mpos, const uint32_t *lidx_p, const uint32_t *lidx_n, EcLiveArc *larc,
                                   uint32_t *no_src)
{
    uint64_t a = (uint64_t) blockIdx.x * blockDim.x + threadIdx.x;
    if (a >= n_arc || arc_del[a]) return;
    const uint64_t w = arc_w[a];
    if (vtx_hs_off[w >> 1] == EC_NO_SRC) *no_src = 1u;
    EcLiveArc x;
    x.w = (uint32_t) w, x.ls = arc_ls[a], x.hs16 = (uint32_t) (vtx_hs_off[w >> 1] >> 4), x.mpos = vtx_mpos[w >> 1];
    x.lp = lidx_p[w], x.ln = lidx_n[w], x.pad[0] = x.pad[1] = 0;
    larc[live_off[a]] = x;
}

struct EcAssembleArgs {
    EcReads rd;
    const uint8_t *scm_del;
    const uint64_t *scm_s;
    const uint64_t *blk_off;
    const EcBlockOut *out;
    const uint64_t *path_pool;
    uint32_t *new_n;
    const uint64_t *new_off;
    uint64_t *new_k_mer, *new_s_mer;
    uint32_t *new_m_pos;
    uint32_t *key_id;
    uint64_t *val_occ;
    uint64_t sid0;
    const uint64_t *old_s_mer;
    unsigned long long *stats;
    int pass;
};

__device__ __forceinline__ uint32_t ecr_u32(uint32_t v, int lane) { return (uint32_t) __builtin_amdgcn_readfirstlane((int32_t) __shfl((int32_t) v, lane)); }
__device__ __forceinline__ uint64_t ecr_u64(uint64_t v, int lane) { return (uint64_t) ecr_u32((uint32_t) (v >> 32), lane) << 32 | ecr_u32((uint32_t) v, lane); }
__device__ __forceinline__ uint64_t ecr_above(int32_t j) { return j < 0? ~0ULL : (j >= 63? 0ULL : ~0ULL << (j + 1)); }

template <class FB, class FC>
__device__ int ec_blocks_wave(int lane, int32_t n, uint64_t km, uint32_t mp, bool del, uint32_t hoco_l, int K, FB on_block, FC on_copy)
{
    const bool in = lane < n;
    const uint64_t goodm = __ballot(in && !del && !(km & 1ULL)), delm = __ballot(in && del);
    const uint32_t pos = mp >> 1;
    int32_t beg = -1, end, nb = 0;
    bool updated = true;
    for (;;) {
        uint32_t beg_pos = beg < 1? 0u : ecr_u32(pos, beg - 1) + (uint32_t) K;
        beg_pos += EC_MIN_ERR_SEQ_LEN;
        const uint64_t m = __ballot(pos >= beg_pos) & goodm & ecr_above(beg);
        end = m? (int32_t) __builtin_ctzll(m) : (beg + 1 < n? n : beg + 1);
        if (beg >= 0 || end < n) {
            EcBlock b;
            if (beg < 0) {
                beg = end;
                const uint64_t kb = ecr_u64(km, beg);
                const uint32_t mb = ecr_u32(mp, beg);
                b.beg_utg = (kb & ~1ULL) | (uint64_t) !(mb & 1u);
                b.beg_pos = 0, b.end_utg = EC_NONE, b.l = (int32_t) (mb >> 1), b.r = 1;
            } else {
                --beg;
                const uint64_t kb = ecr_u64(km, beg);
                const uint32_t mb = ecr_u32(mp, beg);
                b.beg_utg = (kb & ~1ULL) | (mb & 1u);
                b.beg_pos = (mb >> 1) + (uint32_t) K;
                if (end >= n) b.end_utg = EC_NONE, b.l = (int32_t) hoco_l - (int32_t) b.beg_pos;
                else {
                    const uint64_t ke = ecr_u64(km, end);
                    const uint32_t me = ecr_u32(mp, end);
                    b.end_utg = (ke & ~1ULL) | (me & 1u), b.l = (int32_t) (me >> 1) - (int32_t) b.beg_pos;
                }
                b.r = 0;
            }
            b.beg = beg, b.end = end;
            on_block(nb, b);
            ++nb;
        } else {
            updated = false;
        }
        if (end + 1 < n) {
            if (ecr_u64(km, end) & 1ULL) beg = end + 1;
            else { const uint64_t m2 = delm & ecr_above(end); beg = m2? (int32_t) __builtin_ctzll(m2) : n; }
        } else {
            beg = end + 1;
        }
        if (beg > n) break;
        on_copy(end, beg);
    }
    return updated? nb : -1;
}

#ifndef ECR_RPW
#define ECR_RPW 1
#endif
#define ECR_READS_PER_BLOCK (4 * ECR_RPW)

struct EcrRead {
    uint64_t r, o;
    int32_t n;
    uint64_t km;
    uint32_t mp, hoco_l;
    bool del;
};
__device__ __forceinline__ void ecr_load(const EcReads &rd, const uint8_t *scm_del, uint64_t r0, int lane, EcrRead (&q)[ECR_RPW])
{
#pragma unroll
    for (int k = 0; k < ECR_RPW; ++k) {
        q[k].r = r0 + k;
        const bool live = q[k].r < rd.n_reads;
        q[k].o = live? rd.scm_off[q[k].r] : 0;
        q[k].n = live? (int32_t) (rd.scm_off[q[k].r + 1] - q[k].o) : -1;
        q[k].hoco_l = live? rd.hoco_l[q[k].r] : 0;
    }
#pragma unroll
    for (int k = 0; k < ECR_RPW; ++k) {
        const bool in = q[k].n >= 0 && q[k].n <= 64 && lane < q[k].n;
        q[k].km = in? rd.k_mer[q[k].o + lane] : 0;
        q[k].mp = in? rd.m_pos[q[k].o + lane] : 0;
    }
#pragma unroll
    for (int k = 0; k < ECR_RPW; ++k) q[k].del = q[k].n >= 0 && q[k].n <= 64 && lane < q[k].n && scm_del[q[k].km >> 1];
}

__global__ __launch_bounds__(256) void ec_count_blocks_wave_kernel(EcReads rd, const uint8_t *scm_del, uint32_t *n_blocks)
{
    const uint64_t r0 = ((uint64_t) blockIdx.x * 4 + (threadIdx.x >> 6)) * ECR_RPW;
    const int lane = threadIdx.x & 63;
    if (r0 >= rd.n_reads) return;
    EcrRead q[ECR_RPW];
    ecr_load(rd, scm_del, r0, lane, q);
#pragma unroll
    for (int k = 0; k < ECR_RPW; ++k) {
        const EcrRead &x = q[k];
        if (x.n < 0) continue;
        int nb = 0;
        if (x.n > 64) {
            if (lane == 0) {
                ec_blocks(scm_del, rd.k_mer + x.o, rd.m_pos + x.o, x.n, x.hoco_l, rd.K, [&](int, const EcBlock &) { ++nb; }, [](int32_t, int32_t) {});
                n_blocks[x.r] = (uint32_t) nb;
            }
            continue;
        }
        ec_blocks_wave(lane, x.n, x.km, x.mp, x.del, x.hoco_l, rd.K, [&](int, const EcBlock &) { ++nb; }, [](int32_t, int32_t) {});
        if (lane == 0) n_blocks[x.r] = (uint32_t) nb;
    }
}

__global__ __launch_bounds__(256) void ec_list_blocks_wave_kernel(EcReads rd, EcLive lv, const uint8_t *scm_del, const uint64_t *blk_off, EcWork *work, uint32_t *copy_n)
{
    const uint64_t r0 = ((uint64_t) blockIdx.x * 4 + (threadIdx.x >> 6)) * ECR_RPW;
    const int lane = threadIdx.x & 63;
    if (r0 >= rd.n_reads) return;
    EcrRead q[ECR_RPW];
    ecr_load(rd, scm_del, r0, lane, q);
    EcWork *wq[ECR_RPW];
    uint32_t hq[ECR_RPW];
#pragma unroll
    for (int k = 0; k < ECR_RPW; ++k) wq[k] = q[k].n >= 0? work + blk_off[q[k].r] : nullptr, hq[k] = q[k].n >= 0? (uint32_t) (rd.off[q[k].r] >> 6) : 0u;
#pragma unroll
    for (int k = 0; k < ECR_RPW; ++k) {
        const EcrRead &x = q[k];
        if (x.n < 0) continue;
        EcWork *w = wq[k];
        const uint32_t hs16 = hq[k];
        const int32_t n = x.n;
        auto put = [&](int i, const EcBlock &b) {
            EcWork y;
            y.beg_utg = b.beg_utg, y.end_utg = b.end_utg, y.read = (uint32_t) x.r, y.beg_pos = b.beg_pos, y.l = b.l, y.r = b.r;
            y.hs16 = hs16, y.lp = lv.idx_p[b.beg_utg], y.ln = lv.idx_n[b.beg_utg];
            const int32_t last = b.end < n? b.end : n;
            y.pad = b.r? (uint32_t) b.beg : (b.beg + 1 < n && last > b.beg + 1? (uint32_t) (last - b.beg - 1) : 0u);
            w[i] = y;
        };
        uint32_t cp = 0;
        auto on_copy = [&](int32_t first, int32_t last) { if (last > first) cp += (uint32_t) (last - first); };
        if (x.n > 64) {
            if (lane == 0) {
                const int nbs = ec_blocks(scm_del, rd.k_mer + x.o, rd.m_pos + x.o, x.n, x.hoco_l, rd.K, put, on_copy);
                copy_n[x.r] = nbs < 0? (uint32_t) n : cp;
            }
            continue;
        }
        EcBlock mine;
        mine.beg_utg = 0, mine.end_utg = 0, mine.beg_pos = 0, mine.l = 0, mine.beg = 0, mine.end = 0, mine.r = 0;
        const int nb = ec_blocks_wave(lane, x.n, x.km, x.mp, x.del, x.hoco_l, rd.K,
                                      [&](int i, const EcBlock &b) { if (i < 64) { if (lane == i) mine = b; } else if (lane == 0) put(i, b); }, on_copy);
        if (lane < nb) put(lane, mine);
        if (lane == 0) copy_n[x.r] = nb < 0? (uint32_t) n : cp;
    }
}

__global__ __launch_bounds__(256) void ec_new_n_kernel(uint64_t n_reads, const uint32_t *copy_n, const uint64_t *blk_off, const EcWork *work, const EcBlockOut *out, uint32_t *new_n)
{
    const uint64_t r = (uint64_t) blockIdx.x * blockDim.x + threadIdx.x;
    if (r >= n_reads) return;
    uint32_t s = copy_n[r];
    for (uint64_t i = blk_off[r]; i < blk_off[r + 1]; ++i) {
        if (out[i].status == EC_SUCCESS) {
            const int32_t np = (int32_t) out[i].np;
            s += work[i].r? (uint32_t) (np >= 1? np - 1 : 0) : (uint32_t) ((np >= 2? np - 2 : 0) + (work[i].end_utg == EC_NONE && np > 1? 1 : 0));
        } else s += work[i].pad;
    }
    new_n[r] = s;
}

__global__ __launch_bounds__(256) void ec_block_stats_kernel(const EcWork *work, const EcBlockOut *out, uint64_t n_work, unsigned long long *stats)
{
    __shared__ uint32_t part[4][11];
    uint32_t loc[11] = {0, 0, 0, 0, 0, 0, 0, 0, 0, 0, 0};
    for (uint64_t i = (uint64_t) blockIdx.x * blockDim.x + threadIdx.x; i < n_work; i += (uint64_t) gridDim.x * blockDim.x) {
        const EcBlockOut x = out[i];
        if (x.short_block) ++loc[10];
        else if (work[i].end_utg == EC_NONE) ++loc[0], ++loc[1 + x.status];
        else ++loc[5], ++loc[6 + x.status];
    }
    for (int i = 0; i < 11; ++i) {
        uint32_t v = loc[i];
        for (int d = 32; d; d >>= 1) v += __shfl_xor(v, d);
        if ((threadIdx.x & 63) == 0) part[threadIdx.x >> 6][i] = v;
    }
    __syncthreads();
    if (threadIdx.x < 11) {
        const uint32_t v = part[0][threadIdx.x] + part[1][threadIdx.x] + part[2][threadIdx.x] + part[3][threadIdx.x];
        if (v) atomicAdd(&stats[threadIdx.x], (unsigned long long) v);
    }
}

__device__ inline void ec_assemble_read_serial(const EcAssembleArgs &a, uint64_t r)
{
    const uint64_t o = a.rd.scm_off[r];
    const int32_t n = (int32_t) (a.rd.scm_off[r + 1] - o);
    const uint64_t *km = a.rd.k_mer + o;
    const uint32_t *mp = a.rd.m_pos + o;
    const EcBlockOut *bo = a.out + a.blk_off[r];
    uint64_t wpos = a.pass? a.new_off[r] : 0;
    const uint64_t w0 = wpos;
    uint32_t cnt = 0;
    auto put = [&](uint64_t k, uint32_t m) {
        if (a.pass) {
            a.new_k_mer[wpos] = k, a.new_m_pos[wpos] = m, a.new_s_mer[wpos] = a.scm_s[k >> 1];
            a.key_id[wpos] = (uint32_t) (k >> 1), a.val_occ[wpos] = (a.sid0 + r) << 32 | (wpos - w0) << 1 | (m & 1u);
            ++wpos;
        }
        ++cnt;
    };
    int nb = ec_blocks(a.scm_del, km, mp, n, a.rd.hoco_l[r], a.rd.K,
        [&](int k, const EcBlock &b) {
            const EcBlockOut &x = bo[k];
            if (x.status == EC_SUCCESS) {
                const uint64_t *path = a.path_pool + x.path_off;
                const int32_t np = (int32_t) x.np;
                if (b.r) {
                    for (int32_t j = np - 1; j > 0; --j) put((path[j] & ~1ULL) | 1ULL, 0xFFFFFFFFu ^ (uint32_t) (path[j] & 1ULL));
                } else {
                    int32_t j;
                    for (j = 1; j < np - 1; ++j) put((path[j] & ~1ULL) | 1ULL, 0xFFFFFFFEu | (uint32_t) (path[j] & 1ULL));
                    if (b.end_utg == EC_NONE && np > 1) put((path[j] & ~1ULL) | 1ULL, 0xFFFFFFFEu | (uint32_t) (path[j] & 1ULL));
                }
            } else if (b.r) {
                for (int32_t j = 0; j < b.beg; ++j) put(km[j], mp[j]);
            } else if (b.beg + 1 < n) {
                for (int32_t j = b.beg + 1; j < b.end; ++j) put(km[j], mp[j]);
            }
        },
        [&](int32_t first, int32_t last) { for (int32_t j = first; j < last; ++j) put(km[j], mp[j]); });
    if (nb < 0) {
        if (a.pass) {
            uint64_t q = a.new_off[r];
            for (int32_t j = 0; j < n; ++j) {
                a.new_k_mer[q + j] = km[j], a.new_m_pos[q + j] = mp[j], a.new_s_mer[q + j] = a.old_s_mer[o + j];
                a.key_id[q + j] = (uint32_t) (km[j] >> 1), a.val_occ[q + j] = (a.sid0 + r) << 32 | (uint64_t) j << 1 | (mp[j] & 1u);
            }
        }
        cnt = (uint32_t) n;
    }
    if (!a.pass) a.new_n[r] = cnt;
}

template <int PASS>
__global__ __launch_bounds__(256) void ec_assemble_wave_kernel(EcAssembleArgs a)
{
    const uint64_t r0 = ((uint64_t) blockIdx.x * 4 + (threadIdx.x >> 6)) * ECR_RPW;
    const int lane = threadIdx.x & 63;
    if (r0 >= a.rd.n_reads) return;
    EcrRead q[ECR_RPW];
    ecr_load(a.rd, a.scm_del, r0, lane, q);
    const EcBlockOut *boq[ECR_RPW];
    uint32_t st_q[ECR_RPW], np_q[ECR_RPW];
    uint64_t path_q[ECR_RPW], w0_q[ECR_RPW], s_q[ECR_RPW];
#pragma unroll
    for (int k = 0; k < ECR_RPW; ++k) {
        const bool live = q[k].n >= 0;
        const uint64_t b0 = live? a.blk_off[q[k].r] : 0;
        const int32_t nbk = live? (int32_t) (a.blk_off[q[k].r + 1] - b0) : 0;
        boq[k] = a.out + b0;
        st_q[k] = EC_FAILURE, np_q[k] = 0, path_q[k] = 0;
        if (lane < nbk) st_q[k] = boq[k][lane].status, np_q[k] = boq[k][lane].np, path_q[k] = boq[k][lane].path_off;
        w0_q[k] = PASS && live? a.new_off[q[k].r] : 0;
        s_q[k] = PASS && live && q[k].n <= 64 && lane < q[k].n? a.old_s_mer[q[k].o + lane] : 0;
    }
#pragma unroll
    for (int k = 0; k < ECR_RPW; ++k) {
        const EcrRead &x = q[k];
        if (x.n < 0) continue;
        if (x.n > 64) {
            if (lane == 0) ec_assemble_read_serial(a, x.r);
            continue;
        }
        const int32_t n = x.n;
        const uint64_t km = x.km, my_s = s_q[k], w0 = w0_q[k], my_path = path_q[k];
        const uint32_t mp = x.mp, my_status = st_q[k], my_np = np_q[k];
        const EcBlockOut *bo = boq[k];
        uint64_t wpos = w0;
        const uint64_t sid = (a.sid0 + x.r) << 32;
        auto write = [&](uint64_t at, uint64_t kk, uint32_t m, uint64_t sv) {
            a.new_k_mer[at] = kk, a.new_m_pos[at] = m, a.new_s_mer[at] = sv;
            a.key_id[at] = (uint32_t) (kk >> 1), a.val_occ[at] = sid | (at - w0) << 1 | (m & 1u);
        };
        auto copy = [&](int32_t first, int32_t last) {
            if (last <= first) return;
            if (PASS && lane >= first && lane < last) write(wpos + (uint32_t) (lane - first), km, mp, my_s);
            wpos += (uint32_t) (last - first);
        };
        const int nb = ec_blocks_wave(lane, n, km, mp, x.del, x.hoco_l, a.rd.K,
            [&](int i, const EcBlock &b) {
                const uint32_t status = i < 64? ecr_u32(my_status, i) : bo[i].status;
                if (status == EC_SUCCESS) {
                    const int32_t np = (int32_t) (i < 64? ecr_u32(my_np, i) : bo[i].np);
                    const uint64_t *path = a.path_pool + (i < 64? ecr_u64(my_path, i) : bo[i].path_off);
                    int32_t c;
                    if (b.r) c = np >= 1? np - 1 : 0;
                    else c = (np >= 2? np - 2 : 0) + (b.end_utg == EC_NONE && np > 1? 1 : 0);
                    if (PASS) {
                        for (int32_t t = lane; t < c; t += 64) {
                            const uint64_t p = b.r? path[np - 1 - t] : path[1 + t];
                            const uint64_t kk = (p & ~1ULL) | 1ULL;
                            write(wpos + (uint32_t) t, kk, b.r? 0xFFFFFFFFu ^ (uint32_t) (p & 1ULL) : 0xFFFFFFFEu | (uint32_t) (p & 1ULL), a.scm_s[kk >> 1]);
                        }
                    }
                    wpos += (uint32_t) c;
                } else if (b.r) {
                    copy(0, b.beg);
                } else if (b.beg + 1 < n) {
                    copy(b.beg + 1, b.end < n? b.end : n);
                }
            },
            copy);
        if (nb < 0) {
            wpos = w0;
            if (PASS && lane < n) write(w0 + (uint32_t) lane, km, mp, my_s);
            wpos += (uint32_t) n;
        }
        if (!PASS && lane == 0) a.new_n[x.r] = (uint32_t) (wpos - w0);
    }
}

__global__ void ec_fwd_flag_kernel(uint64_t tot, const uint64_t *occ, uint32_t *flag)
{
    uint64_t i = (uint64_t) blockIdx.x * blockDim.x + threadIdx.x;
    if (i < tot) flag[i] = !(occ[i] & 1ULL);
}
__global__ void ec_cov_sorted_kernel(uint64_t tot, const uint32_t *key_sorted, const uint32_t *fwd_incl, uint32_t *cov, uint32_t *fwd)
{
    uint64_t i = (uint64_t) blockIdx.x * blockDim.x + threadIdx.x;
    if (i >= tot) return;
    const uint32_t k = key_sorted[i];
    if (i + 1 < tot && key_sorted[i + 1] == k) return;
    uint64_t lo = 0, hi = i;
    while (lo < hi) {
        const uint64_t mid = (lo + hi) >> 1;
        if (key_sorted[mid] < k) lo = mid + 1; else hi = mid;
    }
    cov[k] = (uint32_t) (i - lo + 1);
    fwd[k] = fwd_incl[i] - (lo? fwd_incl[lo - 1] : 0u);
}

__global__ void ec_del_kernel(uint64_t n, const uint32_t *fwd, uint8_t *del)
{
    uint64_t i = (uint64_t) blockIdx.x * blockDim.x + threadIdx.x;
    if (i < n) del[i] = !fwd[i];
}

}
```

oatk_amd/csrc/ecgraph.hpp:

```cpp
#pragma once
#include "common.hpp"

namespace oatk {

#define EGR_INVALID 0xFFFFFFFFFFFFFFFFULL

__global__ void egr_pair_keys_kernel(uint64_t n_reads, const uint64_t *scm_off, const uint64_t *k_mer, const uint32_t *m_pos, uint64_t *keys, uint32_t *dist,
                                     int skip_corrected = 0)
{
    uint64_t r = (uint64_t) blockIdx.x * blockDim.x + threadIdx.x;
    if (r >= n_reads) return;
    const uint64_t o = scm_off[r], n = scm_off[r + 1] - o;
    if (n == 0) return;
    keys[o] = EGR_INVALID, dist[o] = 0;
    uint64_t v0 = (k_mer[o] >> 1) << 1 | (m_pos[o] & 1u);
    uint32_t p0 = m_pos[o] >> 1;
    for (uint64_t j = 1; j < n; ++j) {
        const uint64_t v1 = (k_mer[o + j] >> 1) << 1 | (m_pos[o + j] & 1u);
        const uint32_t p1 = m_pos[o + j] >> 1;
        keys[o + j] = skip_corrected && ((k_mer[o + j - 1] | k_mer[o + j]) & 1ULL)? EGR_INVALID : (v0 <= v1? v0 << 32 | v1 : (v1 ^ 1ULL) << 32 | (v0 ^ 1ULL));
        dist[o + j] = p1 - p0;
        v0 = v1, p0 = p1;
    }
}

__global__ __launch_bounds__(256) void egr_pair_light_wave_kernel(uint64_t n_reads, const uint64_t *scm_off, const uint64_t *k_mer, const uint32_t *m_pos, const uint32_t *cov,
                                                                  uint32_t c, uint64_t *keys, uint32_t *dist, uint8_t *keep, uint8_t *other)
{
    const uint64_t r = (uint64_t) blockIdx.x * 4 + (threadIdx.x >> 6);
    const int lane = threadIdx.x & 63;
    if (r >= n_reads) return;
    const uint64_t o = scm_off[r];
    const int64_t n = (int64_t) (scm_off[r + 1] - o);
    auto emit = [&](uint64_t at, uint64_t v0, uint32_t p0, uint64_t v1, uint32_t p1) {
        const bool c0 = cov[v0 >> 1] >= c, c1 = cov[v1 >> 1] >= c;
        const uint64_t a = v0 <= v1? v0 : v1 ^ 1ULL, b = v0 <= v1? v1 : v0 ^ 1ULL;
        keys[at] = a << 32 | b, dist[at] = p1 - p0, keep[at] = c0 && c1;
        const bool ca = v0 <= v1? c0 : c1, cb = v0 <= v1? c1 : c0;
        if (ca && !cb) other[a] = 1;
        if (cb && !ca) other[b ^ 1ULL] = 1;
    };
    if (n > 64) {
        if (lane == 0) {
            keys[o] = EGR_INVALID, dist[o] = 0, keep[o] = 0;
            uint64_t v0 = (k_mer[o] >> 1) << 1 | (m_pos[o] & 1u);
            uint32_t p0 = m_pos[o] >> 1;
            for (int64_t j = 1; j < n; ++j) {
                const uint64_t v1 = (k_mer[o + j] >> 1) << 1 | (m_pos[o + j] & 1u);
                const uint32_t p1 = m_pos[o + j] >> 1;
                emit(o + j, v0, p0, v1, p1);
                v0 = v1, p0 = p1;
            }
        }
        return;
    }
    const bool in = lane < n;
    const uint64_t km = in? k_mer[o + lane] : 0;
    const uint32_t mp = in? m_pos[o + lane] : 0;
    const uint64_t v1 = (km >> 1) << 1 | (mp & 1u);
    const uint32_t p1 = mp >> 1;
    const uint64_t v0 = (uint64_t) __shfl_up((long long) v1, 1);
    const uint32_t p0 = (uint32_t) __shfl_up((int) p1, 1);
    if (in && lane == 0) keys[o] = EGR_INVALID, dist[o] = 0, keep[o] = 0;
    if (in && lane > 0) emit(o + lane, v0, p0, v1, p1);
}

__global__ void egr_seg_head_kernel(uint64_t n, const uint64_t *skeys, const uint32_t *sdist, uint8_t *head)
{
    const uint64_t i = (uint64_t) blockIdx.x * blockDim.x + threadIdx.x;
    if (i < n) head[i] = i == 0 || skeys[i] != skeys[i - 1] || sdist[i] != sdist[i - 1];
}
__global__ void egr_seg_emit_kernel(uint64_t n_seg, uint64_t n, const uint32_t *head_pos, const uint64_t *skeys, const uint32_t *sdist, uint64_t *okey, uint64_t *oval)
{
    const uint64_t i = (uint64_t) blockIdx.x * blockDim.x + threadIdx.x;
    if (i >= n_seg) return;
    const uint64_t p = head_pos[i], q = i + 1 < n_seg? head_pos[i + 1] : n;
    okey[i] = skeys[p], oval[i] = (uint64_t) sdist[p] | (q - p) << 32;
}
__global__ void egr_seg_split_kernel(uint64_t n, const uint64_t *val, uint32_t *dist, uint32_t *wgt)
{
    const uint64_t i = (uint64_t) blockIdx.x * blockDim.x + threadIdx.x;
    if (i < n) dist[i] = (uint32_t) val[i], wgt[i] = (uint32_t) (val[i] >> 32);
}

__global__ void egr_expand_count_kernel(uint64_t n_keys, const uint64_t *ukeys, uint32_t *n_out)
{
    uint64_t i = (uint64_t) blockIdx.x * blockDim.x + threadIdx.x;
    if (i >= n_keys) return;
    const uint64_t k = ukeys[i];
    if (k == EGR_INVALID) { n_out[i] = 0; return; }
    const uint64_t v0 = k >> 32, v1 = k & 0xFFFFFFFFULL;
    n_out[i] = (v1 ^ 1ULL) != v0? 2u : 1u;
}

__global__ void egr_expand_kernel(uint64_t n_keys, const uint64_t *ukeys, const uint32_t *counts, const uint32_t *run_ls, const uint64_t *out_off,
                                  uint64_t *akey, uint64_t *aval)
{
    uint64_t i = (uint64_t) blockIdx.x * blockDim.x + threadIdx.x;
    if (i >= n_keys) return;
    const uint64_t k = ukeys[i];
    if (k == EGR_INVALID) return;
    const uint64_t v0 = k >> 32, v1 = k & 0xFFFFFFFFULL, o = out_off[i];
    const uint64_t ls = (v1 ^ 1ULL) == v0? 0ULL : (uint64_t) run_ls[i];
    const uint64_t c = ls << 44 | (uint64_t) counts[i] << 1;
    akey[o] = k, aval[o] = c;
    if ((v1 ^ 1ULL) != v0) akey[o + 1] = (v1 ^ 1ULL) << 32 | (v0 ^ 1ULL), aval[o + 1] = c | 1ULL;
}

struct EgrArcs {
    uint64_t n_arc;
    uint64_t *arc_v, *arc_w;
    uint32_t *arc_ls, *arc_cov;
    uint8_t *arc_comp, *arc_del;
    uint64_t *idx_p;
    uint32_t *idx_n;
    uint32_t *flags;
};

__global__ void egr_unpack_kernel(EgrArcs a, const uint64_t *skey, const uint64_t *sval)
{
    uint64_t i = (uint64_t) blockIdx.x * blockDim.x + threadIdx.x;
    if (i >= a.n_arc) return;
    const uint64_t k = skey[i], v = k >> 32, w = k & 0xFFFFFFFFULL;
    a.arc_v[i] = v, a.arc_w[i] = w;
    a.arc_cov[i] = (uint32_t) (sval[i] >> 1);
    uint8_t comp = (uint8_t) (sval[i] & 1ULL);
    if ((w ^ 1ULL) == v) comp ^= 1;
    a.arc_comp[i] = comp, a.arc_del[i] = 0, a.arc_ls[i] = (uint32_t) (sval[i] >> 44);
    if (i && skey[i - 1] == k) a.flags[0] = 1u;
    if (i == 0 || (skey[i - 1] >> 32) != v) a.idx_p[v] = i;
    atomicAdd(&a.idx_n[v], 1u);
}

struct MiniKh {
    uint32_t bits, count;
    uint64_t used;
    int32_t keys[64], vals[64];
    bool overflow;

    __device__ static uint32_t h2b(uint32_t hash, uint32_t bits) { return (hash * 2654435769U) >> (32 - bits); }
    __device__ void init() { bits = 0, count = 0, used = 0, overflow = false; }
    __device__ uint32_t nb() const { return bits? 1U << bits : 0U; }
    __device__ void resize(uint32_t want)
    {
        uint32_t j = 0, x = want;
        while ((x >>= 1) != 0) ++j;
        if (want & (want - 1)) ++j;
        const uint32_t nbits = j > 2? j : 2;
        if (nbits > 6) { overflow = true; return; }
        const uint32_t n_old = nb(), n_new = 1U << nbits;
        uint64_t nused = 0;
        for (j = 0; j != n_old; ++j) {
            if (!((used >> j) & 1ULL)) continue;
            int32_t key = keys[j], val = vals[j];
            used &= ~(1ULL << j);
            for (;;) {
                uint32_t i = h2b((uint32_t) key, nbits);
                while ((nused >> i) & 1ULL) i = (i + 1) & (n_new - 1);
                nused |= 1ULL << i;
                if (i < n_old && ((used >> i) & 1ULL)) {
                    const int32_t tk = keys[i], tv = vals[i];
                    keys[i] = key, vals[i] = val, key = tk, val = tv;
                    used &= ~(1ULL << i);
                } else {
                    keys[i] = key, vals[i] = val;
                    break;
                }
            }
        }
        used = nused, bits = nbits;
    }
    __device__ void add1(int32_t key)
    {
        uint32_t n = nb();
        if (count >= (n >> 1) + (n >> 2)) { resize(n + 1U); if (overflow) return; n = nb(); }
        uint32_t i = h2b((uint32_t) key, bits);
        const uint32_t last = i;
        while (((used >> i) & 1ULL) && keys[i] != key) { i = (i + 1U) & (n - 1); if (i == last) break; }
        if (!((used >> i) & 1ULL)) keys[i] = key, vals[i] = 1, used |= 1ULL << i, ++count;
        else ++vals[i];
    }
    __device__ void addw(int32_t key, uint32_t w)
    {
        add1(key);
        if (w < 2 || overflow) return;
        add1(key);
        if (w < 3 || overflow) return;
        const uint32_t n = nb();
        uint32_t i = h2b((uint32_t) key, bits);
        while (keys[i] != key || !((used >> i) & 1ULL)) i = (i + 1U) & (n - 1);
        vals[i] += (int32_t) (w - 2);
    }
    __device__ int32_t mode() const
    {
        int32_t movl = 0, mcnt = 0;
        for (uint32_t k = 0; k < nb(); ++k) if (((used >> k) & 1ULL) && vals[k] > mcnt) mcnt = vals[k], movl = keys[k];
        return movl;
    }
};

struct WaveKh {
    int32_t *keys, *vals;
    uint64_t used;
    uint32_t bits, count;
    bool overflow;

    __device__ void init(int32_t *k, int32_t *v) { keys = k, vals = v, used = 0, bits = 0, count = 0, overflow = false; }
    __device__ uint32_t nb() const { return bits? 1U << bits : 0U; }
    __device__ bool due() const { const uint32_t n = nb(); return count >= (n >> 1) + (n >> 2); }
    __device__ void resize(uint32_t want)
    {
        uint32_t j = 0, x = want;
        while ((x >>= 1) != 0) ++j;
        if (want & (want - 1)) ++j;
        const uint32_t nbits = j > 2? j : 2;
        if (nbits > 6) { overflow = true; return; }
        const uint32_t n_old = nb(), n_new = 1U << nbits;
        uint64_t nused = 0;
        for (j = 0; j != n_old; ++j) {
            if (!((used >> j) & 1ULL)) continue;
            int32_t key = keys[j], val = vals[j];
            used &= ~(1ULL << j);
            for (;;) {
                uint32_t i = MiniKh::h2b((uint32_t) key, nbits);
                while ((nused >> i) & 1ULL) i = (i + 1) & (n_new - 1);
                nused |= 1ULL << i;
                if (i < n_old && ((used >> i) & 1ULL)) {
                    const int32_t tk = keys[i], tv = vals[i];
                    keys[i] = key, vals[i] = val, key = tk, val = tv;
                    used &= ~(1ULL << i);
                } else {
                    keys[i] = key, vals[i] = val;
                    break;
                }
            }
        }
        used = nused, bits = nbits;
    }
    __device__ bool add(int32_t key, int32_t cnt)
    {
        for (int pass = 0; pass < 2; ++pass) {
            uint32_t n = nb(), i = 0;
            bool found = false;
            if (n) {
                i = MiniKh::h2b((uint32_t) key, bits);
                const uint32_t last = i;
                while (((used >> i) & 1ULL) && keys[i] != key) { i = (i + 1U) & (n - 1); if (i == last) break; }
                found = (used >> i) & 1ULL;
            }
            if (due()) {
                resize(n + 1U);
                if (overflow) return false;
                continue;
            }
            if (found) { vals[i] += cnt; return false; }
            keys[i] = key, vals[i] = cnt, used |= 1ULL << i, ++count;
            return true;
        }
        return false;
    }
    __device__ int32_t mode() const
    {
        int32_t movl = 0, mcnt = 0;
        for (uint32_t k = 0; k < nb(); ++k) if (((used >> k) & 1ULL) && vals[k] > mcnt) mcnt = vals[k], movl = keys[k];
        return movl;
    }
};

#define EGR_SMALL_RUN 48
#define EGR_HUGE_SCRATCH (256ull << 20)

__device__ __forceinline__ uint32_t egr_to_ls(int64_t l, int K)
{
    if (l < K) l = l < 0? K : K - l;
    else l = 0;
    return (uint32_t) l;
}

__global__ __launch_bounds__(64) void egr_mode_kernel(uint64_t n_runs, const uint64_t *ukeys, const uint32_t *counts, const uint64_t *run_off,
                                                      const uint32_t *sdist, int K, uint32_t *run_ls, uint32_t *flags, uint32_t *big_list, uint32_t *huge_list,
                                                      const uint32_t *swgt = nullptr, uint32_t *run_cov = nullptr)
{
    const int lane = threadIdx.x;
    const uint64_t i = (uint64_t) blockIdx.x * 64 + lane;
    const bool valid = i < n_runs && ukeys[i] != EGR_INVALID;
    const uint32_t c = valid? counts[i] : 0u;
    const uint64_t o = valid? run_off[i] : 0;
    if (valid && c <= EGR_SMALL_RUN) {
        MiniKh h;
        h.init();
        if (swgt) {
            uint32_t tot = 0;
            for (uint32_t t = 0; t < c; ++t) h.addw((int32_t) sdist[o + t], swgt[o + t]), tot += swgt[o + t];
            run_cov[i] = tot;
        } else {
            for (uint32_t t = 0; t < c; ++t) h.add1((int32_t) sdist[o + t]);
        }
        if (h.overflow) huge_list[atomicAdd(&flags[5], 1u)] = (uint32_t) i;
        else run_ls[i] = egr_to_ls(h.mode(), K);
    }
    const bool is_big = valid && c > EGR_SMALL_RUN;
    const uint64_t big = __ballot(is_big);
    if (big) {
        uint32_t base = 0;
        if (lane == __builtin_ctzll(big)) base = atomicAdd(&flags[4], (uint32_t) __builtin_popcountll(big));
        base = (uint32_t) __shfl((int32_t) base, __builtin_ctzll(big));
        if (is_big) big_list[base + (uint32_t) __builtin_popcountll(big & ((1ULL << lane) - 1ULL))] = (uint32_t) i;
    }
}

__global__ __launch_bounds__(64) void egr_mode_big_kernel(const uint32_t *counts, const uint64_t *run_off, const uint32_t *sdist, int K, uint32_t *run_ls,
                                                          uint32_t *flags, const uint32_t *big_list, uint32_t *huge_list, const uint32_t *swgt = nullptr,
                                                          uint32_t *run_cov = nullptr)
{
    __shared__ int32_t tk[64], tv[64];
    const int lane = threadIdx.x;
    const uint32_t n_big = flags[4];
    for (uint32_t b = blockIdx.x; b < n_big; b += gridDim.x) {
        const uint32_t i = big_list[b];
        const uint32_t cc = counts[i];
        const uint64_t oo = run_off[i];
        WaveKh h;
        h.init(tk, tv);
        bool tail_new = false;
        uint32_t tot = 0;
        for (uint32_t t0 = 0; t0 < cc && !h.overflow; t0 += 64) {
            const bool in = t0 + lane < cc;
            const int32_t d = in? (int32_t) sdist[oo + t0 + lane] : 0;
            const uint32_t w = in? (swgt? swgt[oo + t0 + lane] : 1u) : 0u;
            uint64_t rest = __ballot(in);
            while (rest && !h.overflow) {
                const int f = __builtin_ctzll(rest);
                const int32_t x = __builtin_amdgcn_readfirstlane(__shfl(d, f));
                const uint64_t eq = __ballot(in && d == x) & rest;
                rest &= ~eq;
                uint32_t calls = (uint32_t) __builtin_popcountll(eq);
                const uint32_t wf = (uint32_t) __builtin_amdgcn_readfirstlane((int32_t) __shfl(w, f));
                if (swgt) {
                    calls = 0;
                    for (uint64_t q = eq; q; q &= q - 1) calls += (uint32_t) __builtin_amdgcn_readfirstlane((int32_t) __shfl(w, __builtin_ctzll(q)));
                }
                tot += calls;
                const bool fresh = h.add(x, (int32_t) calls);
                tail_new = fresh && eq == (1ULL << f) && t0 + f == cc - 1 && wf == 1u;
            }
        }
        if (!h.overflow && h.due() && !tail_new) h.resize(h.nb() + 1U);
        if (lane == 0) {
            if (swgt && !h.overflow) run_cov[i] = tot;
            if (h.overflow) huge_list[atomicAdd(&flags[5], 1u)] = i;
            else run_ls[i] = egr_to_ls(h.mode(), K);
        }
        __syncthreads();
    }
}

struct BigKh {
    int32_t *keys, *vals;
    uint8_t *used, *nused;
    uint32_t cap, bits, count;
    bool overflow;

    __device__ uint32_t nb() const { return bits? 1U << bits : 0U; }
    __device__ void resize(uint32_t want)
    {
        uint32_t j = 0, x = want;
        while ((x >>= 1) != 0) ++j;
        if (want & (want - 1)) ++j;
        const uint32_t nbits = j > 2? j : 2;
        if (nbits > 30 || (1U << nbits) > cap) { overflow = true; return; }
        const uint32_t n_old = nb(), n_new = 1U << nbits;
        for (j = 0; j != n_new; ++j) nused[j] = 0;
        for (j = 0; j != n_old; ++j) {
            if (!used[j]) continue;
            int32_t key = keys[j], val = vals[j];
            used[j] = 0;
            for (;;) {
                uint32_t i = MiniKh::h2b((uint32_t) key, nbits);
                while (nused[i]) i = (i + 1) & (n_new - 1);
                nused[i] = 1;
                if (i < n_old && used[i]) {
                    const int32_t tk = keys[i], tv = vals[i];
                    keys[i] = key, vals[i] = val, key = tk, val = tv;
                    used[i] = 0;
                } else {
                    keys[i] = key, vals[i] = val;
                    break;
                }
            }
        }
        uint8_t *t = used; used = nused, nused = t;
        bits = nbits;
    }
    __device__ void add1(int32_t key)
    {
        uint32_t n = nb();
        if (count >= (n >> 1) + (n >> 2)) { resize(n + 1U); if (overflow) return; n = nb(); }
        uint32_t i = MiniKh::h2b((uint32_t) key, bits);
        const uint32_t last = i;
        while (used[i] && keys[i] != key) { i = (i + 1U) & (n - 1); if (i == last) break; }
        if (!used[i]) keys[i] = key, vals[i] = 1, used[i] = 1, ++count;
        else ++vals[i];
    }
    __device__ void addw(int32_t key, uint32_t w)
    {
        add1(key);
        if (w < 2 || overflow) return;
        add1(key);
        if (w < 3 || overflow) return;
        const uint32_t n = nb();
        uint32_t i = MiniKh::h2b((uint32_t) key, bits);
        while (keys[i] != key || !used[i]) i = (i + 1U) & (n - 1);
        vals[i] += (int32_t) (w - 2);
    }
    __device__ int32_t mode() const
    {
        int32_t movl = 0, mcnt = 0;
        for (uint32_t k = 0; k < nb(); ++k) if (used[k] && vals[k] > mcnt) mcnt = vals[k], movl = keys[k];
        return movl;
    }
};

__device__ __forceinline__ uint32_t egr_huge_cap(uint32_t c)
{
    uint32_t n = 4;
    while ((uint64_t) n * 3 < (uint64_t) c * 4 + 4 && n < (1U << 30)) n <<= 1;
    return n < (1U << 30)? n << 1 : n;
}

__global__ __launch_bounds__(64) void egr_mode_huge_kernel(const uint32_t *counts, const uint64_t *run_off, const uint32_t *sdist, int K, uint32_t *run_ls,
                                                           uint32_t *flags, const uint32_t *huge_list, uint8_t *scratch, uint64_t scratch_bytes,
                                                           const uint32_t *swgt = nullptr, uint32_t *run_cov = nullptr)
{
    if (threadIdx.x != 0) return;
    const uint32_t n_huge = flags[5];
    for (uint32_t b = blockIdx.x; b < n_huge; b += gridDim.x) {
        const uint32_t i = huge_list[b], cc = counts[i];
        const uint64_t oo = run_off[i];
        const uint32_t cap = egr_huge_cap(cc);
        const uint64_t need = ((uint64_t) cap * 10 + 15) >> 4;
        const uint64_t at = (uint64_t) atomicAdd(&flags[6], (uint32_t) need);
        if (need >= (1ULL << 31) || (at + need) * 16 > scratch_bytes) { flags[1] = 1u; continue; }
        BigKh h;
        uint8_t *base = scratch + at * 16;
        h.keys = (int32_t *) base, h.vals = h.keys + cap, h.used = (uint8_t *) (h.vals + cap), h.nused = h.used + cap;
        h.cap = cap, h.bits = 0, h.count = 0, h.overflow = false;
        uint32_t tot = 0;
        for (uint32_t t = 0; t < cc && !h.overflow; ++t) {
            if (swgt) h.addw((int32_t) sdist[oo + t], swgt[oo + t]), tot += swgt[oo + t];
            else h.add1((int32_t) sdist[oo + t]);
        }
        if (swgt) run_cov[i] = tot;
        if (h.overflow) flags[1] = 1u;
        else run_ls[i] = egr_to_ls(h.mode(), K);
    }
}

__global__ void egr_compact_pairs_kernel(uint64_t n, const uint8_t *keep, const uint32_t *pos, const uint64_t *keys, const uint32_t *dist,
                                         uint64_t *lkeys, uint32_t *ldist, uint64_t *n_out)
{
    const uint64_t i = (uint64_t) blockIdx.x * blockDim.x + threadIdx.x;
    if (i >= n) return;
    const uint32_t k = keep[i], p = pos[i];
    if (k) lkeys[p] = keys[i], ldist[p] = dist[i];
    if (i == n - 1) *n_out = (uint64_t) p + k;
}

}
```

oatk_amd/csrc/kmer_hash.hpp:

```cpp
#pragma once
#include "common.hpp"
#include "count.hpp"

namespace oatk {

struct KmerHashArgs {
    const uint8_t *hoco_s;
    const uint64_t *off;
    uint64_t sid0;
    const uint64_t *rec_lo;
    const uint32_t *rec_mpos;
    uint64_t *rec_hash;
    uint32_t n_rec;
    int K;
};

#define KMH_REC 16
#define KMH_WPL 8

__device__ __forceinline__ uint32_t kmh_rev_in_bytes(uint32_t x)
{
    x = ((x >> 2) & 0x33333333u) | ((x & 0x33333333u) << 2);
    return ((x >> 4) & 0x0F0F0F0Fu) | ((x & 0x0F0F0F0Fu) << 4);
}

#ifndef OATK_KMH_WAVES
#define OATK_KMH_WAVES 8
#endif
__global__ __launch_bounds__(64, OATK_KMH_WAVES) void kmer_hash_kernel(KmerHashArgs a)
{
    extern __shared__ uint64_t kmix[];
    const uint32_t lane = threadIdx.x, rr = lane >> 2, q = lane & 3u;
    const uint32_t base = blockIdx.x * (uint32_t) KMH_REC;
    const int K = a.K;
    const int nbytes = (K - 1) / 4 + 1, nfull = nbytes >> 3, nrem = nbytes & 7, NW = nfull + (nrem? 1 : 0);
    const int stride = NW + 1;
    const uint32_t nrec = a.n_rec - base < (uint32_t) KMH_REC? a.n_rec - base : (uint32_t) KMH_REC;
    if (rr < nrec) {
        const uint32_t mp = a.rec_mpos[base + rr], rev = mp & 1u, pos = mp >> 1;
        const int64_t hsw = (int64_t) (a.off[(a.rec_lo[base + rr] >> 32) - a.sid0] >> 4);
        const uint32_t *hs32 = (const uint32_t *) a.hoco_s;
        uint64_t *out = &kmix[rr * (uint32_t) stride];
        const int per = (NW + 3) >> 2;
        for (int w0 = (int) q * per; w0 < (int) (q + 1) * per && w0 < NW; w0 += KMH_WPL) {
            const int nwd = (int) (q + 1) * per - w0 < KMH_WPL? (int) (q + 1) * per - w0 : KMH_WPL;
            const int n = w0 + nwd > NW? NW - w0 : nwd;
            const int32_t t_lo = rev? (int32_t) pos + K - 32 * (w0 + n) : (int32_t) pos + 32 * w0;
            const int32_t wi = t_lo >> 4;
            const uint32_t sh = ((uint32_t) t_lo & 15u) * 2u;
            uint32_t asc[2 * KMH_WPL + 1];
            const int64_t gbase = hsw + wi;
            if (n == KMH_WPL && gbase >= 0) {
                struct __attribute__((packed, aligned(4))) W4 { uint32_t a, b, c, e; };
                const W4 *src = (const W4 *) (hs32 + gbase);
                const W4 v0 = src[0], v1 = src[1], v2 = src[2], v3 = src[3];
                const uint32_t v4 = hs32[gbase + 16];
                const uint32_t raw[17] = {v0.a, v0.b, v0.c, v0.e, v1.a, v1.b, v1.c, v1.e, v2.a, v2.b, v2.c, v2.e, v3.a, v3.b, v3.c, v3.e, v4};
#pragma unroll
                for (int i = 0; i < 17; ++i) asc[i] = __builtin_bswap32(raw[i]);
            } else {
#pragma unroll
                for (int i = 0; i < 2 * KMH_WPL + 1; ++i) {
                    int64_t gi = gbase + i;
                    gi = gi < 0? 0 : gi;
                    asc[i] = i < 2 * n + 1? __builtin_bswap32(hs32[gi]) : 0u;
                }
            }
#pragma unroll
            for (int c = 0; c < KMH_WPL; ++c) {
                if (c >= n) break;
                const uint32_t x0 = asc[2 * c], x1 = asc[2 * c + 1], x2 = asc[2 * c + 2];
                const uint32_t hi = (uint32_t) (((uint64_t) x0 << 32 | x1) >> (32u - sh));
                const uint32_t lo = (uint32_t) (((uint64_t) x1 << 32 | x2) >> (32u - sh));
                const int j = rev? n - 1 - c : c;
                const int wd = w0 + j;
                int nb = K - 32 * wd;
                nb = nb > 32? 32 : nb;
                uint64_t word;
                if (rev) {
                    uint64_t V = (uint64_t) hi << 32 | lo;
                    if (nb < 32) V &= ~0ULL >> (64 - 2 * nb);
                    const uint64_t R = revcomp32(V);
                    word = nb < 32? bswap64(R & (~0ULL << (64 - 2 * nb)))
                                  : ~((uint64_t) kmh_rev_in_bytes(hi) << 32 | kmh_rev_in_bytes(lo));
                } else {
                    uint64_t V = (uint64_t) hi << 32 | lo;
                    if (nb < 32) V &= ~0ULL << (64 - 2 * nb);
                    word = bswap64(V);
                }
                out[wd] = wd < nfull? murmur_mix_word(word) : word;
            }
        }
    }
    __syncthreads();
    if (lane < nrec) {
        const uint64_t *km = &kmix[lane * (uint32_t) stride];
        uint64_t h = OATK_MURMUR_SEED ^ ((uint64_t) (uint32_t) nbytes * OATK_MURMUR_M);
        for (int wd = 0; wd < nfull; ++wd) h = (h ^ km[wd]) * OATK_MURMUR_M;
        if (nrem) h = (h ^ km[nfull]) * OATK_MURMUR_M;
        h ^= h >> 47; h *= OATK_MURMUR_M; h ^= h >> 47;
        a.rec_hash[base + lane] = h;
    }
}

}
```

Before: 355.8.

## Fuse record compaction, placement and slot packing into kmer hash kernel

Removes the compact_records and place_records kernels and their intermediate rec_* buffers. The kmer hash kernel now reads raw per-shard regions directly over a 2D grid and scatters its hash, position and slot records straight to their final locations, so pack_slots is skipped when slots are already packed. heads_only is folded into a templated pair_sum kernel, and the clus_id minus-one transform passes are folded into the kernels that consume it. Wave intrinsics (readlane, DPP) replace some shuffles in the ec code, and a host sync is dropped. In exchange the grid is sized by the largest shard, so blocks for shorter shards exit early, and the hash kernel does more scattered writes.

```diff
diff --git a/oatk_amd/csrc/api.hip b/oatk_amd/csrc/api.hip
--- a/oatk_amd/csrc/api.hip
+++ b/oatk_amd/csrc/api.hip
@@ -330,11 +330,11 @@
     uint64_t n_reads = 0, seq_bytes = 0, sid0 = 0;
     int K = 0, S = 0;
     bool scanned = false, counted = false;
+    bool slots_packed = false;
 
     DevBuf hoco_l, n_scm, n_nn, n_lrl, ho_rl, hoco_s, nbits;
     DevBuf nn_key, lrl_key, lrl_val, nn_key2, lrl_key2, lrl_val2;
-    DevBuf rec_hash, rec_lo, rec_smer, rec_mpos;
-    DevBuf raw_lo, raw_smer, raw_mpos, shard_cnt, shard_prefix;
+    DevBuf raw_lo, raw_smer, raw_mpos, shard_cnt;
     uint32_t region_cap = 0;
     DevBuf counters;
     uint32_t nn_cap = 0, lrl_cap = 0;
@@ -460,7 +460,7 @@
     (void) hipStreamSynchronize(ctx->stream);
     DevBuf *all[] = {&ctx->in_seq, &ctx->in_off, &ctx->in_len, &ctx->hoco_l, &ctx->n_scm, &ctx->n_nn, &ctx->n_lrl, &ctx->ho_rl,
                      &ctx->hoco_s, &ctx->nbits, &ctx->nn_key, &ctx->lrl_key, &ctx->lrl_val, &ctx->nn_key2, &ctx->lrl_key2,
-                     &ctx->lrl_val2, &ctx->rec_hash, &ctx->rec_lo, &ctx->rec_smer, &ctx->rec_mpos, &ctx->raw_lo, &ctx->raw_smer, &ctx->raw_mpos, &ctx->shard_cnt, &ctx->shard_prefix, &ctx->counters, &ctx->n_scm64,
+                     &ctx->lrl_val2, &ctx->raw_lo, &ctx->raw_smer, &ctx->raw_mpos, &ctx->shard_cnt, &ctx->counters, &ctx->n_scm64,
                      &ctx->scm_off, &ctx->pos_hash, &ctx->pos_lo, &ctx->pos_smer, &ctx->pos_mpos, &ctx->pos_kid, &ctx->key_hash,
                      &ctx->key_sorted, &ctx->iota, &ctx->perm, &ctx->head, &ctx->head_idx, &ctx->newclus, &ctx->clus_id, &ctx->kloc, &ctx->smer_sorted, &ctx->slot_rec, &ctx->scm_loc,
                      &ctx->bad_head, &ctx->tag, &ctx->tmp_perm, &ctx->flags, &ctx->scm_h, &ctx->scm_s, &ctx->scm_cov,
@@ -661,9 +661,9 @@
         uint64_t guess = (seq_bytes / 256 + 1024) / NSH + 256;
         if (ctx->region_cap < guess) ctx->region_cap = (uint32_t) guess;
     }
-    ENSURE(shard_cnt, NSH * 4); ENSURE(shard_prefix, NSH * 8);
+    ENSURE(shard_cnt, NSH * 4);
     uint32_t sc[oatk::OATK_REC_SHARDS];
-    uint64_t spfx[oatk::OATK_REC_SHARDS];
+    uint32_t sc_max = 0;
 
     for (;;) {
         const size_t raw_n = (size_t) ctx->region_cap * NSH;
@@ -682,7 +682,8 @@
         if (c[1] > ctx->lrl_cap) ctx->lrl_cap = c[1] + c[1] / 4, again = true;
         uint64_t tot = 0;
         uint32_t mx = 0;
-        for (uint32_t i = 0; i < NSH; ++i) { spfx[i] = tot; tot += sc[i]; if (sc[i] > mx) mx = sc[i]; }
+        for (uint32_t i = 0; i < NSH; ++i) { tot += sc[i]; if (sc[i] > mx) mx = sc[i]; }
+        sc_max = mx;
         if (mx > ctx->region_cap) ctx->region_cap = mx + mx / 4 + 16, again = true;
         if (tot > 0xFFFFFFF0ULL) { ctx->err = "more than 2^32 syncmer occurrences in one batch"; return OATK_E_ARG; }
         ctx->tot_nn = c[0], ctx->tot_lrl = c[1], ctx->n_occ = tot;
@@ -690,29 +691,7 @@
         ++ctx->retries;
         CK(hipMemsetAsync(ctx->nbits.p, 0, ctx->nbits.cap, ctx->stream));
     }
-    if (ctx->n_occ) {
-        ENSURE(rec_hash, (size_t) ctx->n_occ * 8); ENSURE(rec_lo, (size_t) ctx->n_occ * 8);
-        ENSURE(rec_smer, (size_t) ctx->n_occ * 8); ENSURE(rec_mpos, (size_t) ctx->n_occ * 4);
-        CK(hipMemcpyAsync(ctx->shard_prefix.p, spfx, sizeof(spfx), hipMemcpyHostToDevice, ctx->stream));
-        oatk::CompactArgs ca;
-        ca.raw_lo = ctx->raw_lo.as<uint64_t>(), ca.raw_smer = ctx->raw_smer.as<uint64_t>(), ca.raw_mpos = ctx->raw_mpos.as<uint32_t>();
-        ca.shard_cnt = ctx->shard_cnt.as<uint32_t>(), ca.shard_prefix = ctx->shard_prefix.as<uint64_t>(), ca.region_cap = ctx->region_cap;
-        ca.rec_lo = ctx->rec_lo.as<uint64_t>(), ca.rec_smer = ctx->rec_smer.as<uint64_t>(), ca.rec_mpos = ctx->rec_mpos.as<uint32_t>();
-        hipLaunchKernelGGL(oatk::compact_records_kernel, dim3(NSH), dim3(256), 0, ctx->stream, ca);
-        CK(hipStreamSynchronize(ctx->stream));
-    }
     if (ctx->timing) t_collect(ctx, OATK_T_HPC, OATK_T_SYNCMER_N);
-
-    if (ctx->n_occ) {
-        oatk::KmerHashArgs kh;
-        kh.hoco_s = ctx->hoco_s.as<uint8_t>(), kh.off = ctx->d_off, kh.sid0 = ctx->sid0;
-        kh.rec_lo = ctx->rec_lo.as<uint64_t>(), kh.rec_mpos = ctx->rec_mpos.as<uint32_t>(), kh.rec_hash = ctx->rec_hash.as<uint64_t>();
-        kh.n_rec = (uint32_t) ctx->n_occ, kh.K = ctx->K;
-        const int nw = ((ctx->K - 1) / 4 + 1 + 7) / 8;
-        t_begin(ctx, OATK_T_KMER_HASH);
-        hipLaunchKernelGGL(oatk::kmer_hash_kernel, dim3((unsigned) ((ctx->n_occ + KMH_REC - 1) / KMH_REC)), dim3(64), (size_t) KMH_REC * (nw + 1) * 8, ctx->stream, kh);
-        t_end(ctx, OATK_T_KMER_HASH);
-    }
 
     t_begin(ctx, OATK_T_SCAN_POST);
     ctx->nn_sorted_in_2 = ctx->lrl_sorted_in_2 = false;
@@ -743,28 +722,32 @@
         CK(rocprim::exclusive_scan(ctx->tmp.p, tb, ctx->n_scm64.as<uint64_t>(), ctx->scm_off.as<uint64_t>(), (uint64_t) 0, n_reads + 1,
                                    rocprim::plus<uint64_t>(), ctx->stream));
     }
-    {
-        using namespace oatk;
+    t_end(ctx, OATK_T_SCAN_POST);
+
+    {
         size_t n = ctx->n_occ? ctx->n_occ : 1;
         ENSURE(pos_hash, n * 8); ENSURE(pos_lo, n * 8); ENSURE(pos_smer, n * 8); ENSURE(pos_mpos, n * 4);
-        ENSURE(key_hash, n * 8); ENSURE(iota, n * 4);
-        if (ctx->n_occ) {
-            PlaceArgs p;
-            p.rec_hash = ctx->rec_hash.as<uint64_t>(), p.rec_lo = ctx->rec_lo.as<uint64_t>(), p.rec_smer = ctx->rec_smer.as<uint64_t>();
-            p.rec_mpos = ctx->rec_mpos.as<uint32_t>(), p.n_rec = (uint32_t) ctx->n_occ, p.sid0 = ctx->sid0;
-            p.scm_off = ctx->scm_off.as<uint64_t>(), p.hash_mask = ctx->hash_mask;
-            p.pos_hash = ctx->pos_hash.as<uint64_t>(), p.pos_lo = ctx->pos_lo.as<uint64_t>(), p.pos_smer = ctx->pos_smer.as<uint64_t>();
-            p.pos_mpos = ctx->pos_mpos.as<uint32_t>(), p.key_hash = ctx->key_hash.as<uint64_t>(), p.iota = ctx->iota.as<uint32_t>();
-            t_begin(ctx, OATK_T_COUNT_PLACE);
-            hipLaunchKernelGGL(place_records_kernel, dim3((unsigned) ((ctx->n_occ + 255) / 256)), dim3(256), 0, ctx->stream, p);
-            t_end(ctx, OATK_T_COUNT_PLACE);
-        }
-    }
-    t_end(ctx, OATK_T_SCAN_POST);
+        ENSURE(key_hash, n * 8); ENSURE(iota, n * 4); ENSURE(slot_rec, n * 32);
+    }
+    if (ctx->n_occ) {
+        oatk::KmerHashArgs kh;
+        kh.hoco_s = ctx->hoco_s.as<uint8_t>(), kh.off = ctx->d_off, kh.sid0 = ctx->sid0;
+        kh.raw_lo = ctx->raw_lo.as<uint64_t>(), kh.raw_smer = ctx->raw_smer.as<uint64_t>(), kh.raw_mpos = ctx->raw_mpos.as<uint32_t>();
+        kh.shard_cnt = ctx->shard_cnt.as<uint32_t>(), kh.region_cap = ctx->region_cap;
+        kh.scm_off = ctx->scm_off.as<uint64_t>(), kh.hash_mask = ctx->hash_mask;
+        kh.pos_hash = ctx->pos_hash.as<uint64_t>(), kh.pos_lo = ctx->pos_lo.as<uint64_t>(), kh.pos_smer = ctx->pos_smer.as<uint64_t>();
+        kh.pos_mpos = ctx->pos_mpos.as<uint32_t>(), kh.key_hash = ctx->key_hash.as<uint64_t>(), kh.iota = ctx->iota.as<uint32_t>();
+        kh.slot_rec = ctx->slot_rec.as<uint4>(), kh.K = ctx->K;
+        const int nw = ((ctx->K - 1) / 4 + 1 + 7) / 8;
+        t_begin(ctx, OATK_T_KMER_HASH);
+        hipLaunchKernelGGL(oatk::kmer_hash_kernel, dim3((sc_max + KMH_REC - 1) / KMH_REC, NSH), dim3(64), (size_t) KMH_REC * (nw + 1) * 8, ctx->stream, kh);
+        t_end(ctx, OATK_T_KMER_HASH);
+    }
     CK(hipGetLastError());
     CK(hipStreamSynchronize(ctx->stream));
     if (ctx->timing) { t_collect(ctx, OATK_T_SCAN_POST, OATK_T_COUNT_PLACE); t_collect(ctx, OATK_T_KMER_HASH, OATK_T_KMER_HASH); }
     ctx->scanned = true;
+    ctx->slots_packed = ctx->n_occ != 0;
     return OATK_OK;
 }
 
@@ -782,6 +765,7 @@
 static void scan_reset_downstream(oatk_hip_ctx *ctx)
 {
     ctx->scanned = ctx->counted = false;
+    ctx->slots_packed = false;
     if (ctx->ec) ctx->ec->done = ctx->ec->marked = ctx->ec->graph_resident = ctx->ec->global = false;
     if (ctx->cons) ctx->cons->done = false;
     if (ctx->ag) ctx->ag->done = false;
@@ -965,10 +949,14 @@
     g.flags = ctx->flags.as<uint32_t>();
     ENSURE(slot_rec, n * 32);
     g.slot_rec = ctx->slot_rec.as<uint4>();
-    hipLaunchKernelGGL(pack_slots_kernel, dim3(nb), dim3(256), 0, ctx->stream, g);
-    hipLaunchKernelGGL(pair_sum_kernel, dim3(2048), dim3(256), 0, ctx->stream, ctx->key_hash.as<uint64_t>(), (const uint32_t *) nullptr, (uint32_t) n, ctx->flags.as<uint32_t>(), 8);
-    hipLaunchKernelGGL(pair_sum_kernel, dim3(2048), dim3(256), 0, ctx->stream, ctx->key_sorted.as<uint64_t>(), ctx->perm.as<uint32_t>(), (uint32_t) n, ctx->flags.as<uint32_t>(), 12);
-    hipLaunchKernelGGL(heads_only_kernel, dim3(nb), dim3(256), 0, ctx->stream, g);
+    if (!ctx->slots_packed) {
+        hipLaunchKernelGGL(pack_slots_kernel, dim3(nb), dim3(256), 0, ctx->stream, g);
+        ctx->slots_packed = true;
+    }
+    hipLaunchKernelGGL((pair_sum_kernel<false>), dim3(2048), dim3(256), 0, ctx->stream, ctx->key_hash.as<uint64_t>(), (const uint32_t *) nullptr, (uint32_t) n, ctx->flags.as<uint32_t>(), 8,
+                       (uint32_t *) nullptr, (uint32_t *) nullptr, (uint32_t *) nullptr);
+    hipLaunchKernelGGL((pair_sum_kernel<true>), dim3(2048), dim3(256), 0, ctx->stream, ctx->key_sorted.as<uint64_t>(), ctx->perm.as<uint32_t>(), (uint32_t) n, ctx->flags.as<uint32_t>(), 12,
+                       g.head, g.newclus, g.head_idx);
     {
         size_t tb = 0;
         CK(rocprim::inclusive_scan(nullptr, tb, ctx->head_idx.as<uint32_t>(), ctx->head_idx.as<uint32_t>(), n, rocprim::maximum<uint32_t>(), ctx->stream));
@@ -988,7 +976,7 @@
         n_scm = last_id;
         ENSURE(scm_h, (size_t) n_scm * 8); ENSURE(scm_s, (size_t) n_scm * 8); ENSURE(scm_cov, (size_t) n_scm * 4); ENSURE(scm_loc, (size_t) n_scm * 8);
         ENSURE(scm_occ_off, ((size_t) n_scm + 1) * 8);
-        f.perm = ctx->perm.as<uint32_t>(), f.newclus = ctx->newclus.as<uint32_t>(), f.clus_id = ctx->clus_id.as<uint32_t>(), f.n_rec = (uint32_t) n;
+        f.perm = ctx->perm.as<uint32_t>(), f.newclus = ctx->newclus.as<uint32_t>(), f.clus_id1 = ctx->clus_id.as<uint32_t>(), f.n_rec = (uint32_t) n;
         f.sorted_key = ctx->key_sorted.as<uint64_t>(), f.smer_sorted = ctx->smer_sorted.as<uint64_t>();
         f.loc = ctx->kloc.as<uint64_t>(), f.scm_loc = ctx->scm_loc.as<uint64_t>();
         f.scm_h = ctx->scm_h.as<uint64_t>(), f.scm_s = ctx->scm_s.as<uint64_t>(), f.scm_occ_off = ctx->scm_occ_off.as<uint64_t>();
@@ -999,7 +987,6 @@
     hipLaunchKernelGGL(gather_finish_kernel, dim3(nb), dim3(256), 0, ctx->stream, g, f, ctx->clus_id.as<uint32_t>(), n_scm);
     CK(hipMemsetAsync(ctx->bad_head.p, 0, n * 4, ctx->stream));
     hipLaunchKernelGGL(verify_group_kernel, dim3((unsigned) ((n + 8 * OATK_VG_STRIP - 1) / (8 * OATK_VG_STRIP))), dim3(256), 0, ctx->stream, g, ctx->bad_head.as<uint32_t>());
-    CK(rocprim::transform(ctx->clus_id.as<uint32_t>(), ctx->clus_id.as<uint32_t>(), n, [] __device__(uint32_t v) { return v - 1u; }, ctx->stream));
     uint32_t fl[16];
     CK(hipMemcpyAsync(fl, ctx->flags.p, sizeof(fl), hipMemcpyDeviceToHost, ctx->stream));
     CK(hipStreamSynchronize(ctx->stream));
@@ -1021,7 +1008,6 @@
                            ctx->tag.as<uint32_t>(), ctx->tmp_perm.as<uint32_t>());
         hipLaunchKernelGGL(regather_kernel, dim3(nb), dim3(256), 0, ctx->stream, g);
         { int rc = ids(); if (rc) return rc; }
-        CK(rocprim::transform(ctx->clus_id.as<uint32_t>(), ctx->clus_id.as<uint32_t>(), n, [] __device__(uint32_t v) { return v - 1u; }, ctx->stream));
         hipLaunchKernelGGL(finish_heads_kernel, dim3(nb), dim3(256), 0, ctx->stream, f, n_scm);
     }
     hipLaunchKernelGGL(check_smer_kernel, dim3(nb), dim3(256), 0, ctx->stream, f);
diff --git a/oatk_amd/csrc/common.hpp b/oatk_amd/csrc/common.hpp
--- a/oatk_amd/csrc/common.hpp
+++ b/oatk_amd/csrc/common.hpp
@@ -95,6 +95,10 @@
     return w;
 }
 
+__device__ __forceinline__ int32_t wave_uniform(int32_t v) { return __builtin_amdgcn_readfirstlane(v); }
+__device__ __forceinline__ uint32_t wave_read(uint32_t v, int lane) { return (uint32_t) __builtin_amdgcn_readlane((int32_t) v, wave_uniform(lane)); }
+__device__ __forceinline__ uint32_t wave_prev(uint32_t v) { return (uint32_t) __builtin_amdgcn_update_dpp((int32_t) v, (int32_t) v, 0x138 , 0xf, 0xf, false); }
+
 __device__ __forceinline__ uint32_t wave_incl_sum(uint32_t v, int lane)
 {
 #pragma unroll
diff --git a/oatk_amd/csrc/count.hpp b/oatk_amd/csrc/count.hpp
--- a/oatk_amd/csrc/count.hpp
+++ b/oatk_amd/csrc/count.hpp
@@ -2,56 +2,6 @@
 #include "common.hpp"
 
 namespace oatk {
-
-struct CompactArgs {
-    const uint64_t *raw_lo, *raw_smer;
-    const uint32_t *raw_mpos;
-    const uint32_t *shard_cnt;
-    const uint64_t *shard_prefix;
-    uint32_t region_cap;
-    uint64_t *rec_lo, *rec_smer;
-    uint32_t *rec_mpos;
-};
-
-__global__ __launch_bounds__(256) void compact_records_kernel(CompactArgs a)
-{
-    const uint32_t sh = blockIdx.x, n = a.shard_cnt[sh];
-    const size_t src = (size_t) sh * a.region_cap;
-    const uint64_t dst = a.shard_prefix[sh];
-    for (uint32_t i = threadIdx.x; i < n; i += blockDim.x) {
-        a.rec_lo[dst + i] = a.raw_lo[src + i];
-        a.rec_smer[dst + i] = a.raw_smer[src + i];
-        a.rec_mpos[dst + i] = a.raw_mpos[src + i];
-    }
-}
-
-struct PlaceArgs {
-    const uint64_t *rec_hash, *rec_lo, *rec_smer;
-    const uint32_t *rec_mpos;
-    uint32_t n_rec;
-    uint64_t sid0;
-    const uint64_t *scm_off;
-    uint64_t hash_mask;
-    uint64_t *pos_hash, *pos_lo, *pos_smer;
-    uint32_t *pos_mpos;
-    uint64_t *key_hash;
-    uint32_t *iota;
-};
-
-__global__ void place_records_kernel(PlaceArgs a)
-{
-    uint32_t i = blockIdx.x * blockDim.x + threadIdx.x;
-    if (i >= a.n_rec) return;
-    uint64_t lo = a.rec_lo[i];
-    uint64_t rd = (lo >> 32) - a.sid0;
-    uint64_t p = a.scm_off[rd] + ((uint32_t) lo >> 1);
-    a.pos_hash[p] = a.rec_hash[i];
-    a.key_hash[p] = a.rec_hash[i] & a.hash_mask;
-    a.pos_lo[p] = lo;
-    a.pos_smer[p] = a.rec_smer[i];
-    a.pos_mpos[p] = a.rec_mpos[i];
-    a.iota[p] = (uint32_t) p;
-}
 
 __device__ __forceinline__ uint64_t kmer_word_global(const uint32_t *hs32, uint32_t pos, uint32_t rev, int K, int wd)
 {
@@ -157,7 +107,9 @@
     x *= 0xD6E8FEB86659FD93ULL; x ^= x >> 29; x += key;
     s1 = x;
 }
-__global__ __launch_bounds__(256) void pair_sum_kernel(const uint64_t *key, const uint32_t *perm, uint32_t n, uint32_t *flags, int at)
+template <bool HEADS>
+__global__ __launch_bounds__(256) void pair_sum_kernel(const uint64_t *key, const uint32_t *perm, uint32_t n, uint32_t *flags, int at,
+                                                       uint32_t *head, uint32_t *newclus, uint32_t *head_idx)
 {
     __shared__ uint64_t part[2][4];
     uint64_t s0 = 0, s1 = 0;
@@ -179,6 +131,10 @@
             pair_sums(k[u], v[u], a, b);
             s0 += a, s1 += b;
             if (k[u] < kp[u]) inv = true;
+            if (HEADS) {
+                const uint32_t i = (uint32_t) (i0 + u * stride), h = i == 0 || k[u] != kp[u];
+                head[i] = h, newclus[i] = h, head_idx[i] = h? i : 0u;
+            }
         }
     }
     #pragma unroll
@@ -190,16 +146,6 @@
         atomicAdd((unsigned long long *) (flags + at), (unsigned long long) (part[0][0] + part[0][1] + part[0][2] + part[0][3]));
         atomicAdd((unsigned long long *) (flags + at + 2), (unsigned long long) (part[1][0] + part[1][1] + part[1][2] + part[1][3]));
     }
-}
-
-__global__ void heads_only_kernel(GroupArgs a)
-{
-    uint32_t i = blockIdx.x * blockDim.x + threadIdx.x;
-    if (i >= a.n_rec) return;
-    const uint32_t h = i == 0 || a.sorted_key[i] != a.sorted_key[i - 1];
-    a.head[i] = h;
-    a.newclus[i] = h;
-    a.head_idx[i] = h? i : 0u;
 }
 
 __global__ void mark_heads_kernel(GroupArgs a)
@@ -335,7 +281,7 @@
 struct FinishArgs {
     const uint32_t *perm;
     const uint32_t *newclus;
-    const uint32_t *clus_id;
+    const uint32_t *clus_id1;
     uint32_t n_rec;
     const uint64_t *sorted_key, *smer_sorted;
     uint64_t *scm_h, *scm_s;
@@ -351,7 +297,7 @@
 {
     uint32_t i = blockIdx.x * blockDim.x + threadIdx.x;
     if (i >= a.n_rec) return;
-    uint32_t p = a.perm[i], id = a.clus_id[i];
+    uint32_t p = a.perm[i], id = a.clus_id1[i] - 1u;
     a.pos_kid[p] = (uint64_t) id << 1;
     if (a.newclus[i]) {
         a.scm_h[id] = a.sorted_key[i];
@@ -385,7 +331,7 @@
 {
     uint32_t i = blockIdx.x * blockDim.x + threadIdx.x;
     if (i >= a.n_rec) return;
-    uint32_t id = a.clus_id[i];
+    uint32_t id = a.clus_id1[i] - 1u;
     if (a.smer_sorted[i] != a.scm_s[id]) a.flags[1] = 1u;
 }
 
diff --git a/oatk_amd/csrc/ec.hpp b/oatk_amd/csrc/ec.hpp
--- a/oatk_amd/csrc/ec.hpp
+++ b/oatk_amd/csrc/ec.hpp
@@ -214,13 +214,15 @@
     int pass;
 };
 
-__device__ __forceinline__ uint32_t ecr_u32(uint32_t v, int lane) { return (uint32_t) __builtin_amdgcn_readfirstlane((int32_t) __shfl((int32_t) v, lane)); }
+__device__ __forceinline__ int32_t ecr_s(int32_t v) { return wave_uniform(v); }
+__device__ __forceinline__ uint32_t ecr_u32(uint32_t v, int lane) { return wave_read(v, lane); }
 __device__ __forceinline__ uint64_t ecr_u64(uint64_t v, int lane) { return (uint64_t) ecr_u32((uint32_t) (v >> 32), lane) << 32 | ecr_u32((uint32_t) v, lane); }
 __device__ __forceinline__ uint64_t ecr_above(int32_t j) { return j < 0? ~0ULL : (j >= 63? 0ULL : ~0ULL << (j + 1)); }
 
 template <class FB, class FC>
-__device__ int ec_blocks_wave(int lane, int32_t n, uint64_t km, uint32_t mp, bool del, uint32_t hoco_l, int K, FB on_block, FC on_copy)
-{
+__device__ int ec_blocks_wave(int lane, int32_t n_, uint64_t km, uint32_t mp, bool del, uint32_t hoco_l, int K, FB on_block, FC on_copy)
+{
+    const int32_t n = ecr_s(n_);
     const bool in = lane < n;
     const uint64_t goodm = __ballot(in && !del && !(km & 1ULL)), delm = __ballot(in && del);
     const uint32_t pos = mp >> 1;
@@ -230,7 +232,7 @@
         uint32_t beg_pos = beg < 1? 0u : ecr_u32(pos, beg - 1) + (uint32_t) K;
         beg_pos += EC_MIN_ERR_SEQ_LEN;
         const uint64_t m = __ballot(pos >= beg_pos) & goodm & ecr_above(beg);
-        end = m? (int32_t) __builtin_ctzll(m) : (beg + 1 < n? n : beg + 1);
+        end = ecr_s(m? (int32_t) __builtin_ctzll(m) : (beg + 1 < n? n : beg + 1));
         if (beg >= 0 || end < n) {
             EcBlock b;
             if (beg < 0) {
@@ -265,6 +267,7 @@
         } else {
             beg = end + 1;
         }
+        beg = ecr_s(beg);
         if (beg > n) break;
         on_copy(end, beg);
     }
diff --git a/oatk_amd/csrc/ecgraph.hpp b/oatk_amd/csrc/ecgraph.hpp
--- a/oatk_amd/csrc/ecgraph.hpp
+++ b/oatk_amd/csrc/ecgraph.hpp
@@ -59,8 +59,8 @@
     const uint32_t mp = in? m_pos[o + lane] : 0;
     const uint64_t v1 = (km >> 1) << 1 | (mp & 1u);
     const uint32_t p1 = mp >> 1;
-    const uint64_t v0 = (uint64_t) __shfl_up((long long) v1, 1);
-    const uint32_t p0 = (uint32_t) __shfl_up((int) p1, 1);
+    const uint64_t v0 = (uint64_t) wave_prev((uint32_t) (v1 >> 32)) << 32 | wave_prev((uint32_t) v1);
+    const uint32_t p0 = wave_prev(p1);
     if (in && lane == 0) keys[o] = EGR_INVALID, dist[o] = 0, keep[o] = 0;
     if (in && lane > 0) emit(o + lane, v0, p0, v1, p1);
 }
@@ -304,7 +304,7 @@
     if (big) {
         uint32_t base = 0;
         if (lane == __builtin_ctzll(big)) base = atomicAdd(&flags[4], (uint32_t) __builtin_popcountll(big));
-        base = (uint32_t) __shfl((int32_t) base, __builtin_ctzll(big));
+        base = wave_read(base, __builtin_ctzll(big));
         if (is_big) big_list[base + (uint32_t) __builtin_popcountll(big & ((1ULL << lane) - 1ULL))] = (uint32_t) i;
     }
 }
@@ -331,14 +331,14 @@
             uint64_t rest = __ballot(in);
             while (rest && !h.overflow) {
                 const int f = __builtin_ctzll(rest);
-                const int32_t x = __builtin_amdgcn_readfirstlane(__shfl(d, f));
+                const int32_t x = (int32_t) wave_read((uint32_t) d, f);
                 const uint64_t eq = __ballot(in && d == x) & rest;
                 rest &= ~eq;
                 uint32_t calls = (uint32_t) __builtin_popcountll(eq);
-                const uint32_t wf = (uint32_t) __builtin_amdgcn_readfirstlane((int32_t) __shfl(w, f));
+                const uint32_t wf = wave_read(w, f);
                 if (swgt) {
                     calls = 0;
-                    for (uint64_t q = eq; q; q &= q - 1) calls += (uint32_t) __builtin_amdgcn_readfirstlane((int32_t) __shfl(w, __builtin_ctzll(q)));
+                    for (uint64_t q = eq; q; q &= q - 1) calls += wave_read(w, __builtin_ctzll(q));
                 }
                 tot += calls;
                 const bool fresh = h.add(x, (int32_t) calls);
diff --git a/oatk_amd/csrc/kmer_hash.hpp b/oatk_amd/csrc/kmer_hash.hpp
--- a/oatk_amd/csrc/kmer_hash.hpp
+++ b/oatk_amd/csrc/kmer_hash.hpp
@@ -8,10 +8,18 @@
     const uint8_t *hoco_s;
     const uint64_t *off;
     uint64_t sid0;
-    const uint64_t *rec_lo;
-    const uint32_t *rec_mpos;
-    uint64_t *rec_hash;
-    uint32_t n_rec;
+    const uint64_t *raw_lo;
+    const uint64_t *raw_smer;
+    const uint32_t *raw_mpos;
+    const uint32_t *shard_cnt;
+    uint32_t region_cap;
+    const uint64_t *scm_off;
+    uint64_t hash_mask;
+    uint64_t *pos_hash, *pos_lo, *pos_smer;
+    uint32_t *pos_mpos;
+    uint64_t *key_hash;
+    uint32_t *iota;
+    uint4 *slot_rec;
     int K;
 };
 
@@ -32,13 +40,21 @@
     extern __shared__ uint64_t kmix[];
     const uint32_t lane = threadIdx.x, rr = lane >> 2, q = lane & 3u;
     const uint32_t base = blockIdx.x * (uint32_t) KMH_REC;
+    uint32_t cnt = a.shard_cnt[blockIdx.y];
+    cnt = cnt < a.region_cap? cnt : a.region_cap;
+    if (base >= cnt) return;
+    const size_t src = (size_t) blockIdx.y * a.region_cap + base;
     const int K = a.K;
     const int nbytes = (K - 1) / 4 + 1, nfull = nbytes >> 3, nrem = nbytes & 7, NW = nfull + (nrem? 1 : 0);
     const int stride = NW + 1;
-    const uint32_t nrec = a.n_rec - base < (uint32_t) KMH_REC? a.n_rec - base : (uint32_t) KMH_REC;
+    const uint32_t nrec = cnt - base < (uint32_t) KMH_REC? cnt - base : (uint32_t) KMH_REC;
+    uint64_t lo = 0;
+    uint32_t mp = 0, hsw32 = 0;
     if (rr < nrec) {
-        const uint32_t mp = a.rec_mpos[base + rr], rev = mp & 1u, pos = mp >> 1;
-        const int64_t hsw = (int64_t) (a.off[(a.rec_lo[base + rr] >> 32) - a.sid0] >> 4);
+        mp = a.raw_mpos[src + rr], lo = a.raw_lo[src + rr];
+        const uint32_t rev = mp & 1u, pos = mp >> 1;
+        const int64_t hsw = (int64_t) (a.off[(lo >> 32) - a.sid0] >> 4);
+        hsw32 = (uint32_t) hsw;
         const uint32_t *hs32 = (const uint32_t *) a.hoco_s;
         uint64_t *out = &kmix[rr * (uint32_t) stride];
         const int per = (NW + 3) >> 2;
@@ -92,6 +108,11 @@
             }
         }
     }
+    const int from = (int) (lane & 15u) * 4;
+    const uint64_t my_lo = (uint64_t) (uint32_t) __shfl((int) (lo >> 32), from) << 32 | (uint32_t) __shfl((int) lo, from);
+    const uint32_t my_mp = (uint32_t) __shfl((int) mp, from), my_hsw = (uint32_t) __shfl((int) hsw32, from);
+    uint64_t my_p = 0, my_sm = 0;
+    if (lane < nrec) my_p = a.scm_off[(my_lo >> 32) - a.sid0] + ((uint32_t) my_lo >> 1), my_sm = a.raw_smer[src + lane];
     __syncthreads();
     if (lane < nrec) {
         const uint64_t *km = &kmix[lane * (uint32_t) stride];
@@ -99,7 +120,10 @@
         for (int wd = 0; wd < nfull; ++wd) h = (h ^ km[wd]) * OATK_MURMUR_M;
         if (nrem) h = (h ^ km[nfull]) * OATK_MURMUR_M;
         h ^= h >> 47; h *= OATK_MURMUR_M; h ^= h >> 47;
-        a.rec_hash[base + lane] = h;
+        a.pos_hash[my_p] = h, a.key_hash[my_p] = h & a.hash_mask;
+        a.pos_lo[my_p] = my_lo, a.pos_smer[my_p] = my_sm, a.pos_mpos[my_p] = my_mp, a.iota[my_p] = (uint32_t) my_p;
+        a.slot_rec[2 * (size_t) my_p] = make_uint4((uint32_t) my_lo, (uint32_t) (my_lo >> 32), (uint32_t) my_sm, (uint32_t) (my_sm >> 32));
+        a.slot_rec[2 * (size_t) my_p + 1] = make_uint4(my_mp, my_hsw, 0u, 0u);
     }
 }
 
```

After: 360.1, median of 6. 1.01x the previous value.
